# jmschrei/blueberry

Hardware: AMD Instinct MI355X
Metric: Gpair-updates/s per stress iteration, N=50k (higher is better)
Workload: dtype f32

## Files before the change

blueberry_amd/_lib.py:

```python
import ctypes
import os

_HERE = os.path.dirname(os.path.abspath(__file__))
LIB_PATH = os.environ.get("BB_LIB") or os.path.join(_HERE, "libblueberry_hip.so")

BB_OK, BB_ERR_INVALID, BB_ERR_HIP, BB_ERR_STATE, BB_ERR_NOMEM = 0, 1, 2, 3, 4
BB_F32, BB_F64 = 0, 1
BB_KIND_WISH, BB_KIND_COUNTS = 0, 1
BB_PEER_HANDLE_BYTES = 128

c_i32, c_i64, c_dbl = ctypes.c_int32, ctypes.c_int64, ctypes.c_double
p_i32, p_i64, p_dbl = (ctypes.POINTER(c_i32), ctypes.POINTER(c_i64), ctypes.POINTER(c_dbl))
c_int, c_void_p = ctypes.c_int, ctypes.c_void_p


class LayoutInfo(ctypes.Structure):
    _fields_ = [(name, c_i64) for name in (
        "n_bins", "n_pad", "vw", "rows_per_unit", "units_per_tile", "n_blocks", "n_tiles",
        "n_units")]

    def as_dict(self):
        return {name: int(getattr(self, name)) for name, _ in self._fields_}


SIGNATURES = {
    "bb_version": (c_int, []),
    "bb_last_error": (ctypes.c_char_p, []),
    "bb_device_count": (c_int, [ctypes.POINTER(c_int)]),
    "bb_band_count": (c_int, [p_dbl, c_i64, c_i32, c_i32, c_int, p_i64]),
    "bb_band_count_rows": (c_int, [p_dbl, c_i64, c_i32, c_i32, c_i64, c_i64, c_int, p_i64]),
    "bb_layout_dense_info": (c_int, [c_i64, c_int, ctypes.POINTER(LayoutInfo)]),
    "bb_layout_dense_tiles": (c_int, [c_i64, c_int, p_i32, p_i32, c_i64]),
    "bb_layout_rank_units": (c_int, [c_i64, c_int, c_int, p_i64, p_i64]),
    "bb_solver_create": (c_int, [ctypes.POINTER(c_void_p), c_i64, c_int, c_int, c_int, c_int,
                                 p_i32, p_i32, c_i64]),
    "bb_solver_destroy": (c_int, [c_void_p]),
    "bb_solver_set_stream": (c_int, [c_void_p, c_void_p]),
    "bb_solver_layout": (c_int, [c_void_p, ctypes.POINTER(LayoutInfo), p_i64, p_i64]),
    "bb_solver_set_wish_dense": (c_int, [c_void_p, p_dbl, c_i64, c_int, c_dbl]),
    "bb_solver_set_wish_sparse": (c_int, [c_void_p, p_i64, p_i64, p_dbl, c_i64, c_int, c_dbl,
                                          p_dbl, p_dbl]),
    "bb_triples_create": (c_int, [ctypes.POINTER(c_void_p), p_dbl, c_i64, c_i32, c_i32, c_int]),
    "bb_triples_destroy": (c_int, [c_void_p]),
    "bb_triples_tiles": (c_int, [c_void_p, c_i64, c_int, ctypes.POINTER(ctypes.c_uint8), c_i64]),
    "bb_solver_set_wish_triples": (c_int, [c_void_p, c_void_p, c_int, c_dbl, p_dbl, p_dbl]),
    "bb_solver_set_wish_from_coords": (c_int, [c_void_p, p_dbl]),
    "bb_solver_set_coords": (c_int, [c_void_p, p_dbl]),
    "bb_solver_get_coords": (c_int, [c_void_p, p_dbl]),
    "bb_solver_set_momentum": (c_int, [c_void_p, c_dbl]),
    "bb_solver_iterate": (c_int, [c_void_p, c_i64, c_dbl]),
    "bb_solver_grad": (c_int, [c_void_p]),
    "bb_solver_apply": (c_int, [c_void_p, c_dbl]),
    "bb_comm_unique_id": (c_int, [c_void_p]),
    "bb_solver_comm_init": (c_int, [c_void_p, c_void_p]),
    "bb_solver_allreduce": (c_int, [c_void_p]),
    "bb_solver_iterate_dist": (c_int, [c_void_p, c_i64, c_dbl]),
    "bb_solver_peer_export": (c_int, [c_void_p, c_void_p]),
    "bb_solver_peer_connect": (c_int, [c_void_p, c_void_p]),
    "bb_solver_iterate_peer": (c_int, [c_void_p, c_i64, c_dbl]),
    "bb_solver_peer_status": (c_int, [c_void_p, ctypes.POINTER(c_int)]),
    "bb_solver_peer_set_timeout": (c_int, [c_void_p, c_i64]),
    "bb_solver_peer_form": (c_int, [c_void_p, ctypes.POINTER(c_int)]),
    "bb_solver_peer_set_form": (c_int, [c_void_p, c_int]),
    "bb_group_create": (c_int, [ctypes.POINTER(c_void_p), ctypes.POINTER(c_void_p), c_int]),
    "bb_group_iterate": (c_int, [c_void_p, c_i64, c_dbl]),
    "bb_group_destroy": (c_int, [c_void_p]),
    "bb_solver_comm_world": (c_int, [c_void_p, ctypes.POINTER(c_int)]),
    "bb_solver_comm_abort": (c_int, [c_void_p]),
    "bb_comm_cached": (c_int, [c_int, c_int, c_int, ctypes.POINTER(c_int)]),
    "bb_comm_cached_generation": (c_int, [c_int, c_int, c_int, ctypes.POINTER(c_int),
                                          ctypes.POINTER(ctypes.c_uint64)]),
    "bb_solver_comm_attach": (c_int, [c_void_p]),
    "bb_solver_comm_detach": (c_int, [c_void_p]),
    "bb_comm_cache_clear": (c_int, []),
    "bb_solver_sync_timeout": (c_int, [c_void_p, c_i64]),
    "bb_solver_exchange_size": (c_int, [c_void_p, p_i64]),
    "bb_solver_get_exchange_buffer": (c_int, [c_void_p, ctypes.POINTER(c_void_p)]),
    "bb_solver_set_exchange_buffer": (c_int, [c_void_p, c_void_p]),
    "bb_solver_read_exchange": (c_int, [c_void_p, p_dbl, c_i64]),
    "bb_solver_write_exchange": (c_int, [c_void_p, p_dbl, c_i64]),
    "bb_solver_matvec_sq": (c_int, [c_void_p, p_dbl, p_dbl]),
    "bb_solver_spectral_init": (c_int, [c_void_p, c_int, p_dbl]),
    "bb_solver_spectral_init_tol": (c_int, [c_void_p, c_int, c_dbl, p_dbl, ctypes.POINTER(c_int), p_dbl]),
    "bb_solver_stress": (c_int, [c_void_p, p_dbl]),
    "bb_solver_get_stress_history": (c_int, [c_void_p, p_dbl, c_i64, p_i64]),
    "bb_solver_sync": (c_int, [c_void_p]),
    "bb_solver_set_timing": (c_int, [c_void_p, c_int]),
    "bb_solver_get_timing": (c_int, [c_void_p, p_dbl, p_dbl, p_i64]),
    "bb_solver_get_step_timing": (c_int, [c_void_p, p_dbl]),
    "bb_solver_measure_event_gap": (c_int, [c_void_p, c_int, p_dbl]),
    "bb_solver_measure_stream_read": (c_int, [c_void_p, c_int, p_dbl]),
    "bb_solver_iteration_path": (c_int, [c_void_p, ctypes.POINTER(c_int), ctypes.POINTER(c_int)]),
    "bb_solver_traffic": (c_int, [c_void_p, p_i64, p_i64]),
    "bb_cm_create": (c_int, [ctypes.POINTER(c_void_p), c_i64, c_int]),
    "bb_cm_destroy": (c_int, [c_void_p]),
    "bb_cm_dim": (c_int, [c_void_p, p_i64]),
    "bb_cm_device_ptr": (c_int, [c_void_p, ctypes.POINTER(c_void_p), p_i64, ctypes.POINTER(c_int)]),
    "bb_cm_upload": (c_int, [c_void_p, p_dbl, c_i64]),
    "bb_cm_download": (c_int, [c_void_p, p_dbl, c_i64]),
    "bb_cm_scatter": (c_int, [c_void_p, p_dbl, c_i64, c_i32]),
    "bb_cm_scatter_ex": (c_int, [c_void_p, p_dbl, c_i64, c_i32, c_i32, ctypes.POINTER(ctypes.c_uint8),
                                 ctypes.POINTER(c_i32)]),
    "bb_cm_normalize": (c_int, [c_void_p, c_i64, p_dbl, p_dbl]),
    "bb_cm_marginals": (c_int, [c_void_p, p_dbl]),
    "bb_cm_filter": (c_int, [c_void_p, c_dbl, p_i64, ctypes.POINTER(ctypes.c_uint8)]),
    "bb_cm_symv": (c_int, [c_void_p, p_dbl, p_dbl]),
    "bb_cm_eigenvector": (c_int, [c_void_p, p_dbl, p_dbl, c_dbl, c_i64, p_i64, p_dbl]),
    "bb_cm_correlation": (c_int, [c_void_p, p_dbl]),
    "bb_cm_release_scratch": (c_int, [c_int]),
    "bb_cm_shortest_paths": (c_int, [c_void_p, c_void_p, c_int, c_dbl, p_i64]),
    "bb_cm_balance": (c_int, [c_void_p, c_i64, c_i64, c_i64, c_dbl, c_i64, c_dbl, p_dbl,
                              ctypes.POINTER(ctypes.c_uint8), p_i64, p_dbl]),
    "bb_cm_expected": (c_int, [c_void_p, c_i64, p_dbl, p_dbl, p_i64]),
    "bb_triples_balance": (c_int, [c_void_p, c_i64, c_i64, c_i64, c_dbl, c_i64, c_dbl, p_dbl,
                                   ctypes.POINTER(ctypes.c_uint8), p_i64, p_dbl]),
    "bb_triples_expected": (c_int, [c_void_p, c_i64, p_dbl, p_dbl, p_i64]),
    "bb_triples_pairs": (c_int, [c_void_p, c_i64, p_i64]),
    "bb_binomial_sf": (c_int, [p_i64, c_dbl, p_dbl, p_dbl, c_i64, c_int]),
    "bb_cm_significance": (c_int, [c_void_p, c_i64, c_i64, c_i64, p_dbl, c_dbl, c_dbl, p_dbl, c_dbl,
                                   ctypes.POINTER(c_void_p)]),
    "bb_triples_significance": (c_int, [c_void_p, c_i64, c_i64, c_i64, p_dbl, c_dbl, c_dbl, p_dbl,
                                        c_dbl, ctypes.POINTER(c_void_p)]),
    "bb_sig_size": (c_int, [c_void_p, p_i64, p_i64]),
    "bb_sig_read": (c_int, [c_void_p, p_i32, p_i32, p_dbl, p_dbl]),
    "bb_sig_timing": (c_int, [c_void_p, p_dbl, p_dbl]),
    "bb_sig_destroy": (c_int, [c_void_p]),
    "bb_solver_set_wish_from_cm": (c_int, [c_void_p, c_void_p, c_int, c_dbl]),
    "bb_solver_set_wish_from_cm_block": (c_int, [c_void_p, c_void_p, c_i64, c_int, c_dbl]),
    "bb_solver_set_maps": (c_int, [c_void_p, c_int, p_i64, p_dbl]),
    "bb_solver_set_wish_dense_block": (c_int, [c_void_p, p_dbl, c_i64, c_i64, c_i64, c_int, c_dbl]),
    "bb_solver_stress_maps": (c_int, [c_void_p, p_dbl, c_int]),
    "bb_solver_set_block_steps": (c_int, [c_void_p, p_dbl, c_i64]),
    "bb_solver_set_bin_steps": (c_int, [c_void_p, p_dbl, c_i64]),
    "bb_solver_degrees": (c_int, [c_void_p, p_i64, c_i64]),
    "bb_solver_set_weight_power": (c_int, [c_void_p, c_int]),
    "bb_solver_weight_sums": (c_int, [c_void_p, p_dbl, c_i64]),
    "bb_solver_score": (c_int, [c_void_p, p_dbl, p_dbl, p_dbl]),
    "bb_solver_get_score_timing": (c_int, [c_void_p, p_dbl, p_dbl, p_dbl]),
    "bb_contactmap_scatter": (c_int, [p_dbl, c_i64, c_i32, p_dbl, c_i64, c_int]),
    "bb_contactmap_normalize": (c_int, [p_dbl, c_i64, p_dbl, p_dbl, c_int]),
    "bb_benjamini_hochberg": (c_int, [p_dbl, c_i64, c_i64, p_dbl, c_int]),
    "bb_downsample": (c_int, [ctypes.POINTER(ctypes.c_float), c_i64,
                              ctypes.POINTER(ctypes.c_float), c_i64, c_int]),
}

_lib = None


def load():
    global _lib
    if _lib is not None:
        return _lib
    if not os.path.exists(LIB_PATH):
        raise ImportError(
            "blueberry_amd: %s is missing -- build it with `python -c 'import __graft_entry__ as "
            "g; g.build()'` (or ./build.sh) at the repository root. There is no CPU fallback."
            % LIB_PATH)
    lib = ctypes.CDLL(LIB_PATH)
    for name, (restype, argtypes) in SIGNATURES.items():
        fn = getattr(lib, name)
        fn.restype = restype
        fn.argtypes = argtypes
    _lib = lib
    return lib


def hip_runtimes_loaded():
    paths = set()
    try:
        with open("/proc/self/maps") as fh:
            for line in fh:
                if "libamdhip64" in line:
                    paths.add(line.split()[-1])
    except OSError:
        pass
    return sorted(paths)
# ... 21 lines not shown
```

blueberry_amd/csrc/bb_solver.hip:

```cpp
#include <math.h>
#include <stddef.h>
#include <stdlib.h>
#include <string.h>
#include <time.h>
#include <unistd.h>

#include <algorithm>
#include <cmath>
#include <type_traits>
#include <vector>

#include <condition_variable>
#include <map>
#include <mutex>
#include <thread>
#include <tuple>

#include "bb_comm.h"
#include "bb_common.h"
#include "bb_group_barrier.h"
#include "bb_score.h"
#include "bb_solver_kernels.h"
#include "bb_triples.h"

struct bb_solver {
    int dtype = BB_F32, device = 0, rank = 0, world = 1;
    bool wide = true;
    bb_layout_info L{};
    std::vector<int32_t> tile_I, tile_J;
    int64_t u_begin = 0, u_end = 0, n_local = 0;
    int64_t t_first = 0, n_local_tiles = 0;
    std::vector<int2> udesc;

    hipStream_t stream = nullptr;
    bool own_stream = false;
    bool stream_stuck = false;

    void *d_units = nullptr, *d_X = nullptr, *d_V = nullptr, *d_part = nullptr;
    void *d_exch = nullptr;
    bb::DevBuf own_exch;
    double momentum = 0.0;
    int2 *d_udesc = nullptr;
    int chunk_q = 0, chunk_r = 0;
    bool nontemporal = true;
    bb::DevBuf d_arena;
    int2 *d_wave_slots = nullptr;
    int lds_wave_floats = 0;
    double *d_stresspart = nullptr;
    double *d_stress_slot = nullptr;
    std::vector<int32_t> slot_strip;
    std::vector<int32_t> wave_last_strip;
    int n_maps = 1;
    bb::DevBuf d_bin_scale;
    bb::DevBuf d_map_ptr, d_map_idx;
    bb::DevBuf d_map_scalar;
    std::vector<int64_t> map_begin;
    int64_t *d_red_lists = nullptr;
    int red_stride = 0, red_slices = 0;
    double *d_stress_hist = nullptr, *d_stress_scalar = nullptr;
    double *d_f64_tmp = nullptr;
    bb::DevBuf d_mv_in;
    int64_t rowpart_elems = 0, colpart_elems = 0;
    int n_waves = 0, n_slots = 0;
    int wpb = 4;
    int dense_u0 = -1;
    int defer_cap_units = 0;
    int64_t defer_lds_bytes = 0;
    unsigned defer_attr_done = 0;
    int64_t hist_cap = 0, hist_n = 0;
    bool have_wish = false, have_coords = false, grad_pending = false;
    void *sum_target = nullptr;

    bb::Rccl::Comm comm = nullptr;
    bool comm_cached = false;
    bool comm_suspect = false;

    bb::DevBuf peer_arena;
    int64_t peer_slot_elems = 0, peer_arena_bytes = 0;
    std::vector<void *> peer_mapped;
    std::vector<void *> peer_opened;
    bb::DevBuf d_peer_table;
    bb::DevBuf d_peer_table_x;
    bool peer_fused = true;
    bb::DevBuf d_peer_state;
    int peer_clock_khz = 100000;
    int peer_ranks_on_gpu = 1;
    bb::DevBuf d_peer_mask;
    bb::DevBuf d_peer_counter;
    unsigned long long peer_seq = 0;
    long long peer_limit_ticks = 0;
    bool peer_connected = false;

    bool row_owner = false;
    bool row_owner_built = false;
    bool bin_steps = false;
    int weight_power = 0;
    void *d_full = nullptr, *d_X2 = nullptr;
    int64_t full_ld = 0;
    double *d_ro_part = nullptr;
    int ro_blocks = 0, ro_wpr = 1;
    int64_t ro_launches = 0;

    bool timing = false;
    int timing_stride = 1;
    int64_t timing_iter = 0;
    std::vector<bb::Event> ev;
    size_t ev_used = 0;
    double score_ms[3] = {0.0, 0.0, 0.0};
};

namespace {

void comm_release(bb_solver *s, bool destroy);

constexpr int64_t kHistCap = 1 << 20;
constexpr size_t kMaxTimedLaunches = 4096;

int check_kind_alpha(const char *who, int kind, double alpha) {
    BB_REQUIRE(kind == BB_KIND_WISH || kind == BB_KIND_COUNTS, std::string(who) + ": bad kind");
    BB_REQUIRE(kind == BB_KIND_WISH || alpha > 0.0, std::string(who) + ": alpha must be > 0");
    return BB_OK;
}

hipError_t upload_padded(const bb_solver *s, double *dst, const double *rows, hipStream_t stream) {
    const hipError_t e = hipMemsetAsync(dst, 0, (size_t)s->L.n_pad * 3 * sizeof(double), stream);
    if (e != hipSuccess) return e;
    return hipMemcpyAsync(dst, rows, (size_t)s->L.n_bins * 3 * sizeof(double), hipMemcpyHostToDevice, stream);
}

int enable_peer_access(const char *who, int device) {
    const hipError_t e = hipDeviceEnablePeerAccess(device, 0);
    if (e != hipSuccess && e != hipErrorPeerAccessAlreadyEnabled) return bb::hip_status(who, e);
    (void)hipGetLastError();
    return BB_OK;
}

template <typename TearDown>
int failed_create(int rc, TearDown &&tear_down) {
    const std::string keep = bb_last_error();
    tear_down();
    bb::set_error(keep);
    return rc;
}

int64_t peer_flags_offset(const bb_solver *s) {
    return 2 * (int64_t)s->world * s->peer_slot_elems * bb::elem_size(s->dtype);
}
int64_t peer_xpoison_offset(const bb_solver *s) {
    return peer_flags_offset(s) + bb::round_up((int64_t)s->world * 64, 256);
}
int64_t peer_arena_size(const bb_solver *s) {
    return peer_xpoison_offset(s) + bb::round_up((int64_t)s->world * 64, 256);
}

int waves_per_cu(int64_t n_local) {
    const char *e = getenv("BB_WAVES_PER_CU");
    int v = e ? atoi(e) : (n_local >= 65000 ? 8 : 4);
    if (v < 1) v = 1;
    if (v > 32) v = 32;
    return v;
}

int64_t row_owner_max() {
    const char *e = getenv("BB_ROW_OWNER_MAX");
    return e ? atoll(e) : bb::kRowOwnerMaxBins;
}

int build_indices(bb_solver *s) {
    const int64_t upt = s->L.units_per_tile, vw = s->L.vw;
    const int64_t ch = 3 * vw;
    s->n_local = s->u_end - s->u_begin;
    s->t_first = s->n_local > 0 ? s->u_begin / upt : 0;
    const int64_t t_last = s->n_local > 0 ? (s->u_end - 1) / upt : -1;
    s->n_local_tiles = s->n_local > 0 ? t_last - s->t_first + 1 : 0;

    s->udesc.resize((size_t)std::max<int64_t>(s->n_local, 1));
    for (int64_t ul = 0; ul < s->n_local; ++ul) {
        const int64_t u = s->u_begin + ul, t = u / upt, sub = u % upt;
        s->udesc[ul] = make_int2((int)(s->tile_I[t] * vw + sub * s->L.rows_per_unit),
                                 (int)(s->tile_J[t] * vw));
    }

    int cus = 256;
    hipDeviceGetAttribute(&cus, hipDeviceAttributeMultiprocessorCount, s->device);
    int64_t want = (int64_t)cus * waves_per_cu(s->n_local);
    int64_t nw = std::max<int64_t>(1, std::min<int64_t>(want, s->n_local));
    {
        const char *e = getenv("BB_PAIR");
        const bool pair = !(e && atoi(e) == 0);
        s->wpb = (pair && (s->dtype == BB_F32 || s->wide) && waves_per_cu(s->n_local) >= 8 && nw >= 8)
                     ? 8 : 4;
    }
    nw = bb::round_up(nw, s->wpb);
    s->n_waves = (int)nw;

    if (s->n_local >= ((int64_t)1 << 31))
        return bb::fail(BB_ERR_INVALID, "bb_solver_create: more than 2^31 units on one rank");
    s->nontemporal = s->n_local * bb::kUnitBytes > ((int64_t)240 << 20);
    s->chunk_q = (int)(s->n_local / nw);
    s->chunk_r = (int)(s->n_local % nw);
    std::vector<int2> wave_range(nw);
    int64_t chunk_max = 0;
    for (int64_t w = 0; w < nw; ++w) {
        const int64_t a = w * s->chunk_q + std::min<int64_t>(w, s->chunk_r);
        wave_range[w] = make_int2((int)a, (int)(a + s->chunk_q + (w < s->chunk_r ? 1 : 0)));
        chunk_max = std::max<int64_t>(chunk_max, wave_range[w].y - wave_range[w].x);
    }
    {
        const int64_t wgs_per_cu = std::max<int64_t>(1, (nw / s->wpb + cus - 1) / cus);
        const int64_t budget = 156 * 1024 / wgs_per_cu;
        const int64_t cap = std::min<int64_t>(chunk_max, (budget / s->wpb - 16 - 8) / 48);
        if ((s->dtype == BB_F32 || s->wide) && cap > 0) s->defer_cap_units = (int)cap;
        const int64_t col_words = 3 * vw * bb::elem_size(s->dtype) / 4;
        s->lds_wave_floats = (int)std::max<int64_t>((int64_t)s->defer_cap_units * 12 + 4, col_words);
        s->defer_lds_bytes = (int64_t)s->wpb * s->lds_wave_floats * 4 + 32;
    }
    std::vector<int32_t> &slot_strip = s->slot_strip;
    slot_strip.clear();
    s->wave_last_strip.assign((size_t)nw, -1);
    std::vector<int2> wave_slots(nw);
    for (int64_t w = 0; w < nw; ++w) {
        wave_slots[w] = make_int2((int)slot_strip.size(), -1);
        if (wave_range[w].x >= wave_range[w].y) continue;
        int cur = -1;
        std::vector<int> strips;
        for (int64_t ul = wave_range[w].x; ul < wave_range[w].y; ++ul) {
            const int J = s->udesc[ul].y / (int)vw;
            if (J != cur) { strips.push_back(J); cur = J; }
        }
        for (size_t q = 0; q + 1 < strips.size(); ++q) slot_strip.push_back(strips[q]);
        const int Jlast = strips.back();
        s->wave_last_strip[(size_t)w] = Jlast;
        const bool same_wg = w % s->wpb != 0;
        if (same_wg && wave_slots[w - 1].y >= 0 &&
            slot_strip[(size_t)wave_slots[w - 1].y] == Jlast) {
            wave_slots[w].y = wave_slots[w - 1].y;
        } else {
            wave_slots[w].y = (int)slot_strip.size();
            slot_strip.push_back(Jlast);
        }
    }
    s->n_slots = (int)slot_strip.size();
    s->rowpart_elems = s->n_local_tiles * ch;
    s->colpart_elems = (int64_t)s->n_slots * ch;

    const int64_t nb = s->L.n_blocks;
    std::vector<int64_t> blk_ptr(nb + 1, 0);
    for (int64_t lt = 0; lt < s->n_local_tiles; ++lt) blk_ptr[s->tile_I[s->t_first + lt] + 1]++;
    for (int sl = 0; sl < s->n_slots; ++sl) blk_ptr[slot_strip[sl] + 1]++;
    for (int64_t b = 0; b < nb; ++b) blk_ptr[b + 1] += blk_ptr[b];
    std::vector<int64_t> blk_chunk((size_t)std::max<int64_t>(blk_ptr[nb], 1));
    std::vector<int64_t> fill(blk_ptr.begin(), blk_ptr.end() - 1);
    for (int64_t lt = 0; lt < s->n_local_tiles; ++lt)
        blk_chunk[fill[s->tile_I[s->t_first + lt]]++] = lt * ch;
    for (int sl = 0; sl < s->n_slots; ++sl)
        blk_chunk[fill[slot_strip[sl]]++] = s->rowpart_elems + (int64_t)sl * ch;

    int64_t longest = 0;
    for (int64_t b = 0; b < nb; ++b) longest = std::max(longest, blk_ptr[b + 1] - blk_ptr[b]);
    const int64_t zero_off = s->rowpart_elems + s->colpart_elems;
    const int64_t part_total = zero_off + ch;
    std::vector<int64_t> red_lists;
    {
        s->red_slices = longest <= 64 ? 4 : 8;
        if (const char *f = getenv("BB_REDUCE_SLICES")) s->red_slices = atoi(f) == 4 ? 4 : 8;
        const int64_t quantum = 16 * s->red_slices;
        s->red_stride = (int)bb::round_up(std::max<int64_t>(longest, 1), quantum);
        red_lists.assign((size_t)(nb * s->red_stride), zero_off);
        for (int64_t b = 0; b < nb; ++b)
            for (int64_t k = blk_ptr[b]; k < blk_ptr[b + 1]; ++k)
                red_lists[(size_t)(b * s->red_stride + (k - blk_ptr[b]))] = blk_chunk[k];
    }

    const int64_t es = bb::elem_size(s->dtype);
    s->hist_cap = kHistCap;
    if (s->row_owner) {
        s->full_ld = bb::round_up(s->L.n_bins, s->dtype == BB_F32 ? RowTrip<float>::COLS
                                                                  : RowTrip<double>::COLS);
        s->ro_wpr = s->L.n_bins <= 1024 ? 4 : (s->L.n_bins <= 2048 ? 2 : 1);
        const int rows_per_wg = 4 / s->ro_wpr;
        s->ro_blocks = (int)((s->L.n_bins + rows_per_wg - 1) / rows_per_wg);
// ... 1 lines not shown
    {
        std::vector<std::pair<void **, size_t>> want;
        auto add = [&](auto **ptr, int64_t count) {
            want.push_back({(void **)ptr, (size_t)std::max<int64_t>(count, 1) * sizeof(**ptr)});
        };
        add((char **)&s->d_units, std::max<int64_t>(s->n_local, 1) * bb::kUnitBytes);
        add((char **)&s->d_X, s->L.n_pad * 3 * es);
        add((char **)&s->d_V, s->L.n_pad * 3 * es);
        add((char **)&s->d_part, part_total * es);
        add(&s->d_udesc, (int64_t)s->udesc.size());
        add(&s->d_wave_slots, nw);
        add(&s->d_stresspart, nw);
        add(&s->d_stress_slot, std::max<int64_t>(s->n_slots, 1));
        add(&s->d_red_lists, (int64_t)red_lists.size());
        add(&s->d_stress_hist, kHistCap);
        add(&s->d_stress_scalar, 1);
        add(&s->d_f64_tmp, s->L.n_pad * 3);
        if (s->row_owner) {
            add((char **)&s->d_full, s->L.n_bins * s->full_ld * es);
            add((char **)&s->d_X2, s->L.n_pad * 3 * es);
            add(&s->d_ro_part, 2 * (int64_t)s->ro_blocks);
        }
        size_t total = 0;
        for (auto &w : want) total += (w.second + 255) & ~(size_t)255;
        BB_TRY(bb::alloc_status(s->d_arena, total));
        size_t off = 0;
        for (auto &w : want) {
            *w.first = s->d_arena.as<char>() + off;
            off += (w.second + 255) & ~(size_t)255;
        }
    }
    BB_TRY(bb::alloc_status(s->own_exch, (size_t)((3 * s->L.n_pad + 2) * es)));
    s->d_exch = s->own_exch.p;

    hipStream_t st = s->stream;
    BB_HIP_CHECK(hipMemcpyAsync(s->d_udesc, s->udesc.data(), s->udesc.size() * sizeof(int2),
                                hipMemcpyHostToDevice, st));
    BB_HIP_CHECK(hipMemcpyAsync(s->d_wave_slots, wave_slots.data(), nw * sizeof(int2),
                                hipMemcpyHostToDevice, st));
    BB_HIP_CHECK(hipMemcpyAsync(s->d_red_lists, red_lists.data(),
                                red_lists.size() * sizeof(int64_t), hipMemcpyHostToDevice, st));
    BB_HIP_CHECK(hipMemsetAsync(s->d_part, 0, (size_t)part_total * es, st));
    BB_HIP_CHECK(hipMemsetAsync(s->d_X, 0, (size_t)(s->L.n_pad * 3 * es), st));
    BB_HIP_CHECK(hipMemsetAsync(s->d_V, 0, (size_t)(s->L.n_pad * 3 * es), st));
    if (s->row_owner)
        BB_HIP_CHECK(hipMemsetAsync(s->d_X2, 0, (size_t)(s->L.n_pad * 3 * es), st));
    BB_HIP_CHECK(hipMemsetAsync(s->d_exch, 0, (size_t)((3 * s->L.n_pad + 2) * es), st));
    BB_HIP_CHECK(hipMemsetAsync(s->d_stresspart, 0, (size_t)nw * sizeof(double), st));
    BB_HIP_CHECK(hipMemsetAsync(s->d_stress_slot, 0,
                                (size_t)std::max<int64_t>(s->n_slots, 1) * sizeof(double), st));
    BB_HIP_CHECK(hipStreamSynchronize(st));
    return BB_OK;
}

template <typename TT>
struct TypeTag {
    using T = TT;
};
template <typename TT, bool WW>
struct LayoutTag {
    using T = TT;
    static constexpr bool W = WW;
};

template <typename F>
decltype(auto) by_layout(const bb_solver *s, F &&f) {
    if (s->dtype == BB_F32) return f(LayoutTag<float, true>{});
    if (s->wide) return f(LayoutTag<double, true>{});
    return f(LayoutTag<double, false>{});
}

template <typename F>
decltype(auto) by_dtype(const bb_solver *s, F &&f) {
    if (s->dtype == BB_F32) return f(TypeTag<float>{});
    return f(TypeTag<double>{});
}

template <int V, int... Rest, typename F>
decltype(auto) with_int(int v, F &&f) {
    if constexpr (sizeof...(Rest) == 0) return f(std::integral_constant<int, V>{});
    else return v == V ? f(std::integral_constant<int, V>{}) : with_int<Rest...>(v, f);
}

template <bool NT, int OP, int WPB, typename T, bool W>
int launch_sweep(LayoutTag<T, W>, bb_solver *s, const void *x_in) {
    const auto kern = stress_grad_kernel<T, W, NT, OP, WPB>;
    constexpr unsigned bit = 1u << ((WPB == 8 ? 4 : 0) + (NT ? 2 : 0) + (OP == kOpMatvec2 ? 1 : 0) +
                                    (OP == kOpStressW1 ? 8 : 0) + (OP == kOpStressW2 ? 16 : 0));
    if (s->defer_lds_bytes > 0 && !(s->defer_attr_done & bit)) {
        BB_HIP_CHECK(hipFuncSetAttribute((const void *)kern, hipFuncAttributeMaxDynamicSharedMemorySize,
                                         (int)s->defer_lds_bytes));
        s->defer_attr_done |= bit;
    }
    T *rowpart = (T *)s->d_part +
                 (s->u_begin - s->t_first * s->L.units_per_tile) * (3 * s->L.rows_per_unit);
    T *colpart = (T *)s->d_part + s->rowpart_elems;
    BB_HIP_CHECK(bb::launch(kern, dim3(s->n_waves / s->wpb), dim3(64 * s->wpb), (size_t)s->defer_lds_bytes,
                            s->stream, (const T *)s->d_units, (const T *)x_in, s->d_udesc, s->chunk_q,
                            s->chunk_r, s->d_wave_slots, rowpart, colpart, s->d_stresspart,
                            s->defer_cap_units, s->lds_wave_floats, s->dense_u0, s->d_stress_slot));
    return BB_OK;
}

template <int OP, typename L>
int launch_sweep_op(L lay, bb_solver *s, const void *x_in) {
    constexpr int kPairWpb = sizeof(typename L::T) == 4 || L::W ? 8 : 4;
    return with_int<1, 0>(s->nontemporal ? 1 : 0, [&](auto nt) {
        return with_int<kPairWpb, 4>(s->wpb, [&](auto wpb) {
            return launch_sweep<decltype(nt)::value != 0, OP, decltype(wpb)::value>(lay, s, x_in);
        });
    });
}

constexpr double kScaleGradient = 2.0, kScalePlainSum = 1.0;

template <typename T>
void fill_reduce_params(bb_solver *s, ReduceParams<T> &p, int mode, double lr, double *stress_out,
                        double scale);

template <typename T, bool W>
int launch_exchange_t(LayoutTag<T, W>, bb_solver *s, double lr, double *stress_out, double scale) {
    ReduceParams<T> p;
    fill_reduce_params<T>(s, p, kReducePeer, lr, stress_out, scale);
    const int64_t es = sizeof(T);
    const unsigned segs = 3 * Lay<T, W>::VW / kRedWG;
    const dim3 grid((unsigned)s->L.n_blocks, segs);
    const PeerTableX<T> *xt = s->d_peer_table_x.as<const PeerTableX<T>>() + (s->peer_seq & 1);
    const char *base = s->peer_arena.as<const char>();
    const T *arena = (const T *)(base + (int64_t)(s->peer_seq & 1) * s->world * s->peer_slot_elems * es);
    const unsigned long long *my_poison = (const unsigned long long *)(base + peer_xpoison_offset(s));
    return with_int<4, 8>(s->red_slices, [&](auto slices) -> int {
        constexpr int S = decltype(slices)::value;
        BB_HIP_CHECK(bb::launch(reduce_exchange_kernel<T, W, S>, grid, dim3(128 * S), 0, s->stream, p,
                                (const int64_t *)s->d_red_lists, s->red_stride, xt, arena, my_poison,
                                s->peer_slot_elems, s->d_peer_state.as<PeerState>(),
                                s->peer_limit_ticks));
        return BB_OK;
    });
}

template <typename T>
void fill_reduce_params(bb_solver *s, ReduceParams<T> &p, int mode, double lr, double *stress_out,
                        double scale) {
    p.part = (const T *)s->d_part;
    p.stresspart = s->d_stresspart;
    p.X = s->sum_target ? (T *)s->sum_target : (T *)s->d_X;
    p.V = (T *)s->d_V;
    p.mu = s->sum_target ? T(0) : (T)s->momentum;
    p.scale = (T)scale;
    p.exch = (T *)s->d_exch;
    p.stress_out = stress_out;
    p.n_pad = s->L.n_pad;
    p.n_waves = s->n_waves;
    p.lr = s->sum_target ? T(-1) : (T)lr;
    p.peer = nullptr;
    p.peer_counter = s->d_peer_counter.as<unsigned>();
    p.peer_state = s->d_peer_state.as<PeerState>();
    p.seq = 0;
    p.n_peers = 0;
    if (mode == kReducePeer) {
        p.peer = s->d_peer_table.as<const PeerTable<T>>() + (s->peer_seq & 1);
        p.seq = s->peer_seq;
        p.n_peers = s->world;
    }
    p.mode = mode;
    p.stress_slot = s->d_stress_slot;
    p.n_slots = s->n_slots;
    p.bin_scale = scale == kScalePlainSum ? nullptr : s->d_bin_scale.as<const T>();
    p.map_ptr = s->d_map_ptr.as<int>();
    p.map_idx = s->d_map_idx.as<int>();
    p.n_maps = s->n_maps;
    p.peer_mask = s->d_peer_mask.as<unsigned>();
    p.rank = s->rank;
}

template <typename T, bool W>
int launch_reduce_t(LayoutTag<T, W>, bb_solver *s, int mode, double lr, double *stress_out, double scale) {
    ReduceParams<T> p;
    fill_reduce_params<T>(s, p, mode, lr, stress_out, scale);
    const unsigned segs = 3 * Lay<T, W>::VW / kRedWG;
    const dim3 grid = mode == kReduceStressOnly ? dim3((unsigned)s->n_maps, 1)
// ... 95 lines not shown
            std::max<int64_t>(0, std::min<int64_t>(i_start + rows, n) - i_start);
        const int64_t cols_valid =
            std::max<int64_t>(0, std::min<int64_t>((int64_t)j0 + VW, n) - j0);
        hipError_t e = hipSuccess;
        if (rows_valid < rows || cols_valid < VW)
            e = hipMemsetAsync(stage, 0, (size_t)rows * VW * sizeof(double), s->stream);
        if (e == hipSuccess && rows_valid > 0 && cols_valid > 0)
            e = hipMemcpy2DAsync(stage, VW * sizeof(double), host + (i_start - off) * ld + (j0 - off),
                                 (size_t)ld * sizeof(double), (size_t)cols_valid * sizeof(double),
                                 (size_t)rows_valid, hipMemcpyHostToDevice, s->stream);
        if (e == hipSuccess) {
            e = bb::launch(convert_units_kernel<T, W>, dim3((unsigned)(ue - ul)), dim3(256), 0,
                           s->stream, stage, (T *)s->d_units, s->d_udesc, ul, i_start, n, kind,
                           -1.0 / alpha);
        }
        if (e != hipSuccess)
            rc = bb::hip_status("set_wish_dense", e);
        ul = ue;
    }
    hipError_t e = hipStreamSynchronize(s->stream);
    if (rc == BB_OK && e != hipSuccess)
        rc = bb::hip_status("set_wish_dense", e);
    return rc;
}

int upload_bin_scale(bb_solver *s, const double *padded) {
    const int64_t n = s->L.n_pad, es = bb::elem_size(s->dtype);
    std::vector<char> host((size_t)(n * es));
    for (int64_t i = 0; i < n; ++i) {
        if (s->dtype == BB_F32) ((float *)host.data())[i] = (float)padded[i];
        else ((double *)host.data())[i] = padded[i];
    }
    BB_HIP_CHECK(hipStreamSynchronize(s->stream));
    if (!s->d_bin_scale) BB_TRY(bb::alloc_status(s->d_bin_scale, (size_t)(n * es)));
    BB_HIP_CHECK(hipMemcpy(s->d_bin_scale.p, host.data(), host.size(), hipMemcpyHostToDevice));
    return BB_OK;
}

int refresh_full(bb_solver *s) {
    if (!s->row_owner) return BB_OK;
    const int64_t es = bb::elem_size(s->dtype);
    BB_HIP_CHECK(hipMemsetAsync(s->d_full, 0, (size_t)(s->L.n_bins * s->full_ld * es), s->stream));
    if (s->n_local > 0)
        BB_TRY(by_layout(s, [&](auto lay) -> int {
            using T = typename decltype(lay)::T;
            BB_HIP_CHECK(bb::launch(units_to_full_kernel<T, decltype(lay)::W>, dim3((unsigned)s->n_local),
                                    dim3(256), 0, s->stream, (const T *)s->d_units, s->d_udesc,
                                    (T *)s->d_full, s->full_ld, s->L.n_bins));
            return BB_OK;
        }));
    BB_HIP_CHECK(hipStreamSynchronize(s->stream));
    return BB_OK;
}

int launch_row_owner(bb_solver *s, double lr, bool fold_prev, bool update) {
    const int par = (int)(s->ro_launches & 1);
    const double *prev = s->d_ro_part + (int64_t)(par ^ 1) * s->ro_blocks;
    double *out = s->d_ro_part + (int64_t)par * s->ro_blocks;
    double *hist_prev = fold_prev ? s->d_stress_hist + (s->hist_n - 1) : nullptr;
    const unsigned grid = update ? (unsigned)s->ro_blocks + 1u : 1u;
    BB_TRY(by_dtype(s, [&](auto t) {
        using T = typename decltype(t)::T;
        return with_int<4, 2, 1>(s->ro_wpr, [&](auto wpr) {
            return with_int<1, 2, 0>(s->weight_power, [&](auto q) -> int {
                BB_HIP_CHECK(bb::launch(row_owner_kernel<T, decltype(wpr)::value, decltype(q)::value>,
                                        dim3(grid), dim3(256), 0, s->stream, (const T *)s->d_full,
                                        s->full_ld, (int)s->L.n_bins, (const T *)s->d_X, (T *)s->d_X2,
                                        (T *)s->d_V, (T)lr, (T)s->momentum, prev, s->ro_blocks, hist_prev,
                                        out, s->d_bin_scale.as<const T>()));
                return BB_OK;
            });
        });
    }));
    if (update) {
        std::swap(s->d_X, s->d_X2);
        s->ro_launches++;
    }
    return BB_OK;
}

int inputs_done(bb_solver *s) {
    BB_HIP_CHECK(hipStreamSynchronize(s->stream));
    BB_TRY(refresh_full(s));
    s->have_wish = true;
    return BB_OK;
}

int pack_from_cm(bb_solver *s, const double *m, int64_t d, int64_t off, int kind, double alpha) {
    BB_TRY(bb::enter_device(s->device));
    if (s->n_local > 0)
        BB_TRY(by_layout(s, [&](auto lay) -> int {
            using T = typename decltype(lay)::T;
            BB_HIP_CHECK(bb::launch(pack_units_from_matrix_kernel<T, decltype(lay)::W>,
                                    dim3((unsigned)s->n_local), dim3(256), 0, s->stream, m, d,
                                    (T *)s->d_units, s->d_udesc, off + d, kind, -1.0 / alpha, off));
            return BB_OK;
        }));
    return inputs_done(s);
}

int set_wish_dense(bb_solver *s, const double *host, int64_t ld, int kind, double alpha, int64_t off,
                   int64_t n_sub) {
    BB_TRY(bb::enter_device(s->device));
    BB_TRY(by_layout(s, [&](auto lay) { return set_wish_dense_t(lay, s, host, ld, kind, alpha, off, n_sub); }));
    return inputs_done(s);
}

template <typename Stage>
int scatter_entries(bb_solver *s, const char *who, int64_t n, int64_t chunk, int kind, double alpha,
                    const double *KRnorm, const double *KRexpected, Stage &&stage) {
    const auto hip = [&](hipError_t e) { return bb::hip_status(who, e); };
    const int64_t nb = s->L.n_blocks;
    std::vector<int32_t> tilemap((size_t)(nb * nb), -1);
    for (size_t t = 0; t < s->tile_I.size(); ++t)
        tilemap[(size_t)s->tile_I[t] * nb + s->tile_J[t]] = (int32_t)t;
    bb::DevBuf bmap, bbad, bkr, bke;
    if (bmap.alloc(tilemap.size() * 4) != hipSuccess || bbad.alloc(sizeof(int)) != hipSuccess ||
        (KRnorm && (bkr.alloc((size_t)s->L.n_bins * 8) != hipSuccess ||
                    bke.alloc((size_t)s->L.n_bins * 8) != hipSuccess)))
        return bb::fail(BB_ERR_NOMEM, std::string(who) + ": out of device memory");
    hipStream_t st = s->stream;
    BB_TRY(hip(hipMemcpyAsync(bmap.p, tilemap.data(), tilemap.size() * 4, hipMemcpyHostToDevice, st)));
    if (KRnorm) {
        BB_TRY(hip(hipMemcpyAsync(bkr.p, KRnorm, (size_t)s->L.n_bins * 8, hipMemcpyHostToDevice, st)));
        BB_TRY(hip(hipMemcpyAsync(bke.p, KRexpected, (size_t)s->L.n_bins * 8, hipMemcpyHostToDevice, st)));
    }
    BB_TRY(hip(hipMemsetAsync(bbad.p, 0, sizeof(int), st)));
    BB_TRY(hip(hipMemsetAsync(s->d_units, 0, (size_t)std::max<int64_t>(s->n_local, 1) * bb::kUnitBytes, st)));
    for (int64_t k0 = 0; k0 < n; k0 += chunk) {
        const int64_t m = std::min(chunk, n - k0);
        EntrySrc src;
        BB_TRY(hip(stage(k0, m, &src)));
        for (int ph = 0; ph < 3; ++ph)
            BB_TRY(hip(by_layout(s, [&](auto lay) {
                using T = typename decltype(lay)::T;
                return bb::launch(scatter_entries_kernel<T, decltype(lay)::W>, dim3((unsigned)((m + 255) / 256)),
                                  dim3(256), 0, st, src, m, (const int32_t *)bmap.p, nb, s->L.n_bins,
                                  s->u_begin, s->u_end, (T *)s->d_units, kind, -1.0 / alpha,
                                  (const double *)bkr.p, (const double *)bke.p, (int *)bbad.p, ph);
            })));
    }
    BB_TRY(hip(hipStreamSynchronize(st)));
    int bad = 0;
    BB_TRY(hip(hipMemcpy(&bad, bbad.p, sizeof(int), hipMemcpyDeviceToHost)));
    if (bad == 1)
        return bb::fail(BB_ERR_INVALID, std::string(who) + ": an index is outside [0, n_bins)");
    if (bad == 2)
        return bb::fail(BB_ERR_INVALID, std::string(who) + ": an entry falls in a tile that is not in "
                                                           "the solver's tile list");
    return inputs_done(s);
}

}

namespace {

struct PeerHandle {
    hipIpcMemHandle_t ipc;
    uint64_t magic;
    int64_t arena_bytes, slot_elems;
    int64_t pid;
    uint64_t raw;
    int32_t rank, world, dtype, device;
    uint64_t pci;
};
static_assert(sizeof(PeerHandle) <= BB_PEER_HANDLE_BYTES, "handle blob too small");
static_assert(offsetof(PeerTable<float>, flag) == kMaxPeers * sizeof(void *) &&
                  offsetof(PeerTable<double>, flag) == kMaxPeers * sizeof(void *),
              "peer_receive_kernel takes the flag pointers as the second half of a PeerTable");
constexpr uint64_t kPeerMagic = 0x6262706565723031ull;

int contributor_mask(const bb_solver *s, std::vector<unsigned> *mask) {
    mask->assign((size_t)s->L.n_blocks, 0u);
    const int64_t upt = s->L.units_per_tile;
    for (int q = 0; q < s->world; ++q) {
        int64_t ub = 0, ue = 0;
        BB_TRY(bb_layout_rank_units(s->L.n_units, q, s->world, &ub, &ue));
        if (ue <= ub) continue;
        for (int64_t t = ub / upt; t <= (ue - 1) / upt; ++t) {
            (*mask)[(size_t)s->tile_I[(size_t)t]] |= 1u << q;
            (*mask)[(size_t)s->tile_J[(size_t)t]] |= 1u << q;
        }
    }
    return BB_OK;
}

template <typename T>
int build_peer_tables(TypeTag<T>, bb_solver *s) {
    PeerTable<T> tab[2];
    memset(tab, 0, sizeof(tab));
    const int64_t foff = peer_flags_offset(s);
    for (int par = 0; par < 2; ++par)
        for (int q = 0; q < s->world; ++q) {
            char *base = (char *)s->peer_mapped[q];
            tab[par].dst[q] = (T *)base + ((int64_t)par * s->world + s->rank) * s->peer_slot_elems;
            tab[par].flag[q] = (unsigned long long *)(base + foff) + 8 * s->rank;
        }
    BB_TRY(bb::alloc_status(s->d_peer_table, sizeof(tab)));
    BB_HIP_CHECK(hipMemcpy(s->d_peer_table.p, tab, sizeof(tab), hipMemcpyHostToDevice));
    PeerTableX<T> tx[2];
    memset(tx, 0, sizeof(tx));
    for (int par = 0; par < 2; ++par)
        for (int q = 0; q < s->world; ++q) {
            char *base = (char *)s->peer_mapped[q];
            tx[par].dst[q] = tab[par].dst[q];
            tx[par].poison[q] = (unsigned long long *)(base + peer_xpoison_offset(s)) + 8 * s->rank;
        }
    BB_TRY(bb::alloc_status(s->d_peer_table_x, sizeof(tx)));
    BB_HIP_CHECK(hipMemcpy(s->d_peer_table_x.p, tx, sizeof(tx), hipMemcpyHostToDevice));
// ... 82 lines not shown
        }
    }
    for (void *m : s->peer_opened) hipIpcCloseMemHandle(m);
    const int device = s->device;
    hipStream_t pooled = s->own_stream && !s->stream_stuck ? s->stream : nullptr;
    delete s;
    if (pooled) bb::release_stream(device, pooled);
    (void)hipGetLastError();
    return BB_OK;
}

int bb_solver_set_stream(bb_solver *s, void *hip_stream) {
    BB_REQUIRE(s != nullptr, "bb_solver_set_stream: solver is NULL");
    BB_TRY(bb::enter_device(s->device));
    BB_HIP_CHECK(hipStreamSynchronize(s->stream));
    if (s->own_stream && s->stream) bb::release_stream(s->device, s->stream);
    s->stream = (hipStream_t)hip_stream;
    s->own_stream = false;
    return BB_OK;
}

int bb_solver_layout(const bb_solver *s, bb_layout_info *info, int64_t *u_begin, int64_t *u_end) {
    BB_REQUIRE(s != nullptr, "bb_solver_layout: solver is NULL");
    if (info) *info = s->L;
    if (u_begin) *u_begin = s->u_begin;
    if (u_end) *u_end = s->u_end;
    return BB_OK;
}

int bb_solver_set_wish_dense(bb_solver *s, const double *host, int64_t ld, int kind,
                             double alpha) {
    BB_REQUIRE(s != nullptr && host != nullptr, "bb_solver_set_wish_dense: NULL argument");
    BB_REQUIRE(ld >= s->L.n_bins, "bb_solver_set_wish_dense: ld < n_bins");
    BB_TRY(check_kind_alpha("bb_solver_set_wish_dense", kind, alpha));
    return set_wish_dense(s, host, ld, kind, alpha, 0, s->L.n_bins);
}

int bb_solver_set_maps(bb_solver *s, int n_maps, const int64_t *bin_begin, const double *lr_scale) {
    BB_REQUIRE(s != nullptr && bin_begin != nullptr && lr_scale != nullptr,
               "bb_solver_set_maps: NULL argument");
    BB_REQUIRE(n_maps >= 1 && n_maps <= s->L.n_blocks, "bb_solver_set_maps: bad n_maps");
    if (s->world != 1)
        return bb::fail(BB_ERR_STATE, "bb_solver_set_maps: one rank only (on several GPUs give every "
                                      "rank maps of its own)");
    const int64_t vw = s->L.vw, nb = s->L.n_blocks;
    BB_REQUIRE(bin_begin[0] == 0 && bin_begin[n_maps] == s->L.n_bins,
               "bb_solver_set_maps: bin_begin must run from 0 to n_bins");
    for (int m = 0; m < n_maps; ++m)
        BB_REQUIRE(bin_begin[m] % vw == 0 && bin_begin[m + 1] > bin_begin[m],
                   "bb_solver_set_maps: every map starts at a multiple of the tile edge and is not empty");
    BB_TRY(bb::enter_device(s->device));
    std::vector<int> map_of_block((size_t)nb, 0);
    for (int m = 0, b = 0; b < nb; ++b) {
        while (m + 1 < n_maps && (int64_t)b * vw >= bin_begin[m + 1]) ++m;
        map_of_block[(size_t)b] = m;
    }
    for (size_t t = 0; t < s->tile_I.size(); ++t)
        BB_REQUIRE(map_of_block[(size_t)s->tile_I[t]] == map_of_block[(size_t)s->tile_J[t]],
                   "bb_solver_set_maps: a tile of the solver's list joins two maps");
    std::vector<double> scale((size_t)s->L.n_pad);
    for (int64_t i = 0; i < s->L.n_pad; ++i) scale[(size_t)i] = lr_scale[map_of_block[(size_t)(i / vw)]];
    std::vector<std::vector<int>> lists((size_t)n_maps);
    for (int w = 0; w < s->n_waves; ++w)
        if (s->wave_last_strip[(size_t)w] >= 0)
            lists[(size_t)map_of_block[(size_t)s->wave_last_strip[(size_t)w]]].push_back(w);
    for (int q = 0; q < s->n_slots; ++q)
        lists[(size_t)map_of_block[(size_t)s->slot_strip[(size_t)q]]].push_back(s->n_waves + q);
    std::vector<int> ptr(1, 0), idx;
    for (auto &l : lists) {
        idx.insert(idx.end(), l.begin(), l.end());
        ptr.push_back((int)idx.size());
    }
    if (idx.empty()) idx.push_back(0);
    s->d_bin_scale.reset(); s->d_map_ptr.reset(); s->d_map_idx.reset(); s->d_map_scalar.reset();
    s->bin_steps = false;
    s->n_maps = 1;
    s->map_begin.clear();
    BB_TRY(upload_bin_scale(s, scale.data()));
    BB_TRY(bb::alloc_status(s->d_map_ptr, ptr.size() * sizeof(int)));
    BB_TRY(bb::alloc_status(s->d_map_idx, idx.size() * sizeof(int)));
    BB_TRY(bb::alloc_status(s->d_map_scalar, (size_t)n_maps * sizeof(double)));
    BB_HIP_CHECK(hipMemcpy(s->d_map_ptr.p, ptr.data(), ptr.size() * sizeof(int), hipMemcpyHostToDevice));
    BB_HIP_CHECK(hipMemcpy(s->d_map_idx.p, idx.data(), idx.size() * sizeof(int), hipMemcpyHostToDevice));
    BB_HIP_CHECK(hipMemsetAsync(s->d_units, 0, (size_t)std::max<int64_t>(s->n_local, 1) * bb::kUnitBytes,
                                s->stream));
    BB_HIP_CHECK(hipStreamSynchronize(s->stream));
    s->n_maps = n_maps;
    s->map_begin.assign(bin_begin, bin_begin + n_maps + 1);
    s->row_owner = false;
    s->hist_n = 0;
    return BB_OK;
}

int bb_solver_set_bin_steps(bb_solver *s, const double *scale, int64_t n_bins) {
    BB_REQUIRE(s != nullptr, "bb_solver_set_bin_steps: solver is NULL");
    if (s->n_maps > 1 && scale == nullptr)
        return bb::fail(BB_ERR_STATE, "bb_solver_set_bin_steps: a solver of several maps always has "
                                      "factors (bb_solver_set_maps sets each map's; pass new ones)");
    if (s->grad_pending)
        return bb::fail(BB_ERR_STATE, "bb_solver_set_bin_steps: a bb_solver_grad is pending");
    BB_TRY(bb::enter_device(s->device));
    if (scale == nullptr) {
        BB_HIP_CHECK(hipStreamSynchronize(s->stream));
        s->d_bin_scale.reset();
        s->bin_steps = false;
        return BB_OK;
    }
    BB_REQUIRE(n_bins == s->L.n_bins, "bb_solver_set_bin_steps: one factor per bin");
    std::vector<double> padded((size_t)s->L.n_pad, 1.0);
    for (int64_t i = 0; i < n_bins; ++i) {
        BB_REQUIRE(std::isfinite(scale[i]) && scale[i] > 0.0,
                   "bb_solver_set_bin_steps: factors must be finite and positive");
        padded[(size_t)i] = scale[i];
    }
    BB_TRY(upload_bin_scale(s, padded.data()));
    s->bin_steps = true;
    return BB_OK;
}

int bb_solver_set_block_steps(bb_solver *s, const double *scale, int64_t n_blocks) {
    BB_REQUIRE(s != nullptr, "bb_solver_set_block_steps: solver is NULL");
    if (scale == nullptr) return bb_solver_set_bin_steps(s, nullptr, 0);
    BB_REQUIRE(n_blocks == s->L.n_blocks, "bb_solver_set_block_steps: one factor per block of the "
                                          "layout (bb_solver_layout: n_blocks)");
    std::vector<double> per_bin((size_t)s->L.n_bins);
    for (int64_t i = 0; i < s->L.n_bins; ++i) per_bin[(size_t)i] = scale[i / s->L.vw];
    return bb_solver_set_bin_steps(s, per_bin.data(), s->L.n_bins);
}

int bb_solver_degrees(bb_solver *s, int64_t *degree, int64_t n_bins) {
    BB_REQUIRE(s != nullptr && degree != nullptr, "bb_solver_degrees: NULL argument");
    BB_REQUIRE(n_bins == s->L.n_bins, "bb_solver_degrees: one count per bin");
    if (!s->have_wish) return bb::fail(BB_ERR_STATE, "bb_solver_degrees: no wish distances set");
    BB_TRY(bb::enter_device(s->device));
    int *d_deg = (int *)s->d_f64_tmp;
    BB_HIP_CHECK(hipMemsetAsync(d_deg, 0, (size_t)s->L.n_pad * sizeof(int), s->stream));
    if (s->n_local > 0)
        BB_TRY(by_layout(s, [&](auto lay) -> int {
            using T = typename decltype(lay)::T;
            BB_HIP_CHECK(bb::launch(unit_degrees_kernel<T, decltype(lay)::W>,
                                    dim3((unsigned)((s->n_local + kDegUnits - 1) / kDegUnits)), dim3(256),
                                    0, s->stream, (const T *)s->d_units, s->d_udesc, s->n_local,
                                    s->L.n_bins, d_deg));
            return BB_OK;
        }));
    std::vector<int> host((size_t)n_bins);
    BB_HIP_CHECK(hipStreamSynchronize(s->stream));
    BB_HIP_CHECK(hipMemcpy(host.data(), d_deg, (size_t)n_bins * sizeof(int), hipMemcpyDeviceToHost));
    for (int64_t i = 0; i < n_bins; ++i) degree[i] = host[(size_t)i];
    return BB_OK;
}

int bb_solver_set_weight_power(bb_solver *s, int q) {
    BB_REQUIRE(s != nullptr, "bb_solver_set_weight_power: solver is NULL");
    BB_REQUIRE(q >= 0 && q <= 2, "bb_solver_set_weight_power: q must be 0, 1 or 2");
    if (s->grad_pending)
        return bb::fail(BB_ERR_STATE, "bb_solver_set_weight_power: a bb_solver_grad is pending");
    s->weight_power = q;
    return BB_OK;
}

int bb_solver_weight_sums(bb_solver *s, double *sums, int64_t n_bins) {
    BB_REQUIRE(s != nullptr && sums != nullptr, "bb_solver_weight_sums: NULL argument");
    BB_REQUIRE(n_bins == s->L.n_bins, "bb_solver_weight_sums: one sum per bin");
    if (!s->have_wish) return bb::fail(BB_ERR_STATE, "bb_solver_weight_sums: no wish distances set");
    BB_TRY(bb::enter_device(s->device));
// ... 134 lines not shown

int bb_triples_create(bb_triples **out, const double *triples, int64_t n, int32_t resolution,
                      int32_t row_major, int device) {
    BB_REQUIRE(out != nullptr, "bb_triples_create: out is NULL");
    *out = nullptr;
    BB_REQUIRE(n >= 0 && (n == 0 || triples != nullptr), "bb_triples_create: NULL triples");
    BB_REQUIRE(resolution > 0, "bb_triples_create: resolution must be positive");
    BB_TRY(bb::use_device(device));
    bb_triples *t = new (std::nothrow) bb_triples();
    if (!t) return bb::fail(BB_ERR_NOMEM, "bb_triples_create: out of host memory");
    t->device = device;
    t->n = n;
    t->resolution = (double)resolution;
    if (row_major) { t->st = 3; t->sc = 1; } else { t->st = 1; t->sc = n; }
    int rc = bb::alloc_status(t->d, (size_t)(3 * n) * sizeof(double));
    if (rc == BB_OK && n > 0)
        rc = bb::hip_status("bb_triples_create",
                            hipMemcpy(t->d.p, triples, (size_t)n * 24, hipMemcpyHostToDevice));
    if (rc != BB_OK) {
        delete t;
        return rc;
    }
    *out = t;
    return BB_OK;
}

int bb_triples_destroy(bb_triples *t) {
    if (!t) return BB_OK;
    hipSetDevice(t->device);
    delete t;
    (void)hipGetLastError();
    return BB_OK;
}

int bb_triples_tiles(const bb_triples *t, int64_t n_bins, int dtype, uint8_t *present,
                     int64_t n_blocks) {
    BB_REQUIRE(t != nullptr && present != nullptr, "bb_triples_tiles: NULL argument");
    bb_layout_info L;
    BB_TRY(bb_layout_dense_info(n_bins, dtype, &L));
    BB_REQUIRE(n_blocks == L.n_blocks, "bb_triples_tiles: present must hold n_blocks^2 bytes of "
                                       "the layout of (n_bins, dtype)");
    BB_TRY(bb::enter_device(t->device));
    bb::DevBuf bp, bb_;
    if (bp.alloc((size_t)(n_blocks * n_blocks)) != hipSuccess || bb_.alloc(sizeof(int)) != hipSuccess)
        return bb::fail(BB_ERR_NOMEM, "bb_triples_tiles: out of device memory");
    BB_HIP_CHECK(hipMemset(bp.p, 0, (size_t)(n_blocks * n_blocks)));
    BB_HIP_CHECK(hipMemset(bb_.p, 0, sizeof(int)));
    constexpr int64_t kChunk = (int64_t)1 << 30;
    for (int64_t k0 = 0; k0 < t->n; k0 += kChunk) {
        const int64_t m = std::min(kChunk, t->n - k0);
        const EntrySrc src = {nullptr, nullptr, nullptr, t->from(k0), t->st, t->sc, t->resolution};
        BB_HIP_CHECK(bb::launch(entries_tiles_kernel, dim3((unsigned)((m + 255) / 256)), dim3(256), 0,
                                (hipStream_t) nullptr, src, m, L.vw, n_blocks, n_bins,
                                (unsigned char *)bp.p, (int *)bb_.p));
    }
    int bad = 0;
    BB_HIP_CHECK(hipMemcpy(&bad, bb_.p, sizeof(int), hipMemcpyDeviceToHost));
    BB_HIP_CHECK(hipMemcpy(present, bp.p, (size_t)(n_blocks * n_blocks), hipMemcpyDeviceToHost));
    if (bad) return bb::fail(BB_ERR_INVALID, "bb_triples_tiles: an index is outside [0, n_bins)");
    return BB_OK;
}

int bb_solver_set_wish_triples(bb_solver *s, const bb_triples *t, int kind, double alpha,
                               const double *KRnorm, const double *KRexpected) {
    BB_REQUIRE(s != nullptr && t != nullptr, "bb_solver_set_wish_triples: NULL argument");
    BB_TRY(check_kind_alpha("bb_solver_set_wish_triples", kind, alpha));
    BB_REQUIRE((KRnorm == nullptr) == (KRexpected == nullptr),
               "bb_solver_set_wish_triples: KRnorm and KRexpected go together");
    BB_REQUIRE(t->device == s->device,
               "bb_solver_set_wish_triples: the triples live on another device than the solver");
    BB_TRY(bb::enter_device(s->device));
    constexpr int64_t kChunk = (int64_t)1 << 30;
    return scatter_entries(s, "bb_solver_set_wish_triples", t->n, kChunk, kind, alpha, KRnorm, KRexpected,
                           [&](int64_t k0, int64_t, EntrySrc *src) {
        *src = {nullptr, nullptr, nullptr, t->from(k0), t->st, t->sc, t->resolution};
        return hipSuccess;
    });
}

int bb_solver_set_wish_from_coords(bb_solver *s, const double *xstar) {
    BB_REQUIRE(s != nullptr && xstar != nullptr, "bb_solver_set_wish_from_coords: NULL argument");
    BB_TRY(bb::enter_device(s->device));
    BB_HIP_CHECK(upload_padded(s, s->d_f64_tmp, xstar, s->stream));
    if (s->n_local > 0)
        BB_TRY(by_layout(s, [&](auto lay) -> int {
            using T = typename decltype(lay)::T;
            BB_HIP_CHECK(bb::launch(gen_units_kernel<T, decltype(lay)::W>, dim3((unsigned)s->n_local),
                                    dim3(256), 0, s->stream, s->d_f64_tmp, (T *)s->d_units, s->d_udesc,
                                    s->L.n_bins));
            return BB_OK;
        }));
    return inputs_done(s);
}

int bb_solver_set_coords(bb_solver *s, const double *xyz) {
    BB_REQUIRE(s != nullptr && xyz != nullptr, "bb_solver_set_coords: NULL argument");
    BB_TRY(bb::enter_device(s->device));
    const int64_t n3 = s->L.n_pad * 3;
    BB_HIP_CHECK(upload_padded(s, s->d_f64_tmp, xyz, s->stream));
    BB_HIP_CHECK(narrow(s, s->d_f64_tmp, s->d_X, n3));
    BB_HIP_CHECK(hipMemsetAsync(s->d_V, 0, (size_t)n3 * bb::elem_size(s->dtype), s->stream));
    BB_HIP_CHECK(hipStreamSynchronize(s->stream));
    s->have_coords = true;
    s->hist_n = 0;
    s->grad_pending = false;
    return BB_OK;
}

int bb_solver_get_coords(bb_solver *s, double *xyz) {
    BB_REQUIRE(s != nullptr && xyz != nullptr, "bb_solver_get_coords: NULL argument");
    if (!s->have_coords) return bb::fail(BB_ERR_STATE, "bb_solver_get_coords: no coordinates set");
    BB_TRY(bb::enter_device(s->device));
    const int64_t n3 = s->L.n_pad * 3;
    BB_HIP_CHECK(widen(s, s->d_X, s->d_f64_tmp, n3));
    BB_HIP_CHECK(hipStreamSynchronize(s->stream));
    BB_HIP_CHECK(hipMemcpy(xyz, s->d_f64_tmp, (size_t)s->L.n_bins * 3 * sizeof(double),
                           hipMemcpyDeviceToHost));
    return BB_OK;
}

int bb_solver_set_momentum(bb_solver *s, double mu) {
    BB_REQUIRE(s != nullptr, "bb_solver_set_momentum: solver is NULL");
    BB_REQUIRE(mu >= 0.0 && mu < 1.0, "bb_solver_set_momentum: need 0 <= mu < 1");
    s->momentum = mu;
    return BB_OK;
}

int bb_solver_iterate(bb_solver *s, int64_t iters, double lr) {
    BB_TRY(check_iterate(s, iters, "bb_solver_iterate"));
    if (s->world != 1)
        return bb::fail(BB_ERR_STATE,
                        "bb_solver_iterate: world > 1 needs bb_solver_grad / all-reduce / "
                        "bb_solver_apply");
    BB_TRY(bb::enter_device(s->device));
    if (s->row_owner) {
        for (int64_t k = 0; k < iters; ++k) {
            BB_TRY(timed_step(s, [&] { return launch_row_owner(s, lr, k > 0, true); },
                              [] { return (int)BB_OK; }));
            s->hist_n++;
        }
        if (iters > 0) BB_TRY(launch_row_owner(s, lr, true, false));
        return BB_OK;
    }
    for (int64_t k = 0; k < iters; ++k) {
        BB_TRY(timed_step(s, [&] { return launch_grad(s); }, [&] {
            return launch_reduce(s, kReduceApply, lr, s->d_stress_hist + s->hist_n * s->n_maps);
        }));
        s->hist_n++;
    }
    return BB_OK;
}

int bb_solver_grad(bb_solver *s) {
    BB_TRY(check_ready(s, "bb_solver_grad"));
    if (s->n_maps > 1)
        return bb::fail(BB_ERR_STATE, "bb_solver_grad: a solver of several maps (bb_solver_set_maps) "
                                      "iterates with bb_solver_iterate only");
    BB_TRY(bb::enter_device(s->device));
    BB_TRY(timed_step(s, [&] { return launch_grad(s); },
                      [&] { return launch_reduce(s, kReduceExchange, 0.0, nullptr); }));
    s->grad_pending = true;
    return BB_OK;
}

int bb_solver_apply(bb_solver *s, double lr) {
    BB_TRY(check_ready(s, "bb_solver_apply"));
// ... 296 lines not shown
    h.device = s->device;
    {
        int dom = 0, bus = 0, dev = 0;
        if (hipDeviceGetAttribute(&dom, hipDeviceAttributePciDomainID, s->device) != hipSuccess ||
            hipDeviceGetAttribute(&bus, hipDeviceAttributePciBusId, s->device) != hipSuccess ||
            hipDeviceGetAttribute(&dev, hipDeviceAttributePciDeviceId, s->device) != hipSuccess) {
            (void)hipGetLastError();
            dom = bus = dev = 0;
        }
        h.pci = ((uint64_t)(uint32_t)dom << 32) | ((uint64_t)(bus & 0xffff) << 16) | (uint64_t)(dev & 0xffff);
    }
    memset(handle_out, 0, BB_PEER_HANDLE_BYTES);
    memcpy(handle_out, &h, sizeof(h));
    return BB_OK;
}

int bb_solver_peer_connect(bb_solver *s, const void *handles) {
    BB_REQUIRE(s != nullptr && handles != nullptr, "bb_solver_peer_connect: NULL argument");
    if (!s->peer_arena) return bb::fail(BB_ERR_STATE, "bb_solver_peer_connect: export first");
    if (s->peer_connected) return bb::fail(BB_ERR_STATE, "bb_solver_peer_connect: already connected");
    BB_TRY(bb::enter_device(s->device));
    s->peer_mapped.assign((size_t)s->world, nullptr);
    std::map<uint64_t, int> ranks_on_gpu;
    int most_on_one_gpu = 1;
    for (int r = 0; r < s->world; ++r) {
        PeerHandle h;
        memcpy(&h, (const char *)handles + (size_t)r * BB_PEER_HANDLE_BYTES, sizeof(h));
        most_on_one_gpu = std::max(most_on_one_gpu, ++ranks_on_gpu[h.pci]);
        if (h.magic != kPeerMagic || h.rank != r || h.world != s->world || h.dtype != s->dtype ||
            h.arena_bytes != s->peer_arena_bytes || h.slot_elems != s->peer_slot_elems)
            return bb::fail(BB_ERR_INVALID, "bb_solver_peer_connect: handle " + std::to_string(r) +
                                                " does not match this solver (rank order, world, "
                                                "dtype and n_bins must agree)");
        if (r == s->rank) {
            s->peer_mapped[r] = s->peer_arena.p;
        } else if (h.pid == (int64_t)getpid()) {
            if (h.device != s->device)
                BB_TRY(enable_peer_access("bb_solver_peer_connect: peer access", h.device));
            s->peer_mapped[r] = (void *)(uintptr_t)h.raw;
        } else {
            void *ptr = nullptr;
            hipError_t e = hipIpcOpenMemHandle(&ptr, h.ipc, hipIpcMemLazyEnablePeerAccess);
            if (e != hipSuccess)
                return bb::fail(BB_ERR_HIP, "bb_solver_peer_connect: hipIpcOpenMemHandle(rank " +
                                                std::to_string(r) + "): " + hipGetErrorString(e));
            s->peer_mapped[r] = ptr;
            s->peer_opened.push_back(ptr);
        }
    }
    BB_TRY(by_dtype(s, [&](auto t) { return build_peer_tables(t, s); }));
    {
        const char *env = getenv("BB_PEER_MASK");
        s->d_peer_mask.reset();
        if (!(env && atoi(env) == 0) && s->world <= 32) {
            std::vector<unsigned> mask;
            BB_TRY(contributor_mask(s, &mask));
            BB_TRY(bb::alloc_status(s->d_peer_mask, mask.size() * sizeof(unsigned)));
            BB_HIP_CHECK(hipMemcpy(s->d_peer_mask.p, mask.data(), mask.size() * sizeof(unsigned),
                                   hipMemcpyHostToDevice));
        }
    }
    BB_TRY(bb::alloc_status(s->d_peer_state, sizeof(PeerState)));
    const int64_t n_counters = 32 * (s->L.n_blocks + 1);
    BB_TRY(bb::alloc_status(s->d_peer_counter, (size_t)n_counters * sizeof(unsigned)));
    BB_HIP_CHECK(hipMemset(s->d_peer_state.p, 0, sizeof(PeerState)));
    BB_HIP_CHECK(hipMemset(s->d_peer_counter.p, 0, (size_t)n_counters * sizeof(unsigned)));
    int khz = 0;
    if (hipDeviceGetAttribute(&khz, hipDeviceAttributeWallClockRate, s->device) != hipSuccess) {
        (void)hipGetLastError();
        khz = 0;
    }
    s->peer_clock_khz = khz > 0 ? khz : 100000;
    long long ms = 10000;
    if (const char *env = getenv("BB_PEER_TIMEOUT_MS")) {
        const long long v = atoll(env);
        if (v > 0) ms = v;
    }
    s->peer_limit_ticks = ms * s->peer_clock_khz;
    s->peer_seq = 0;
    {
        const char *env = getenv("BB_PEER_FUSED");
        s->peer_fused = env ? atoi(env) != 0 : most_on_one_gpu == 1;
        s->peer_ranks_on_gpu = most_on_one_gpu;
    }
    s->peer_connected = true;
    BB_HIP_CHECK(hipDeviceSynchronize());
    return BB_OK;
}

int bb_solver_peer_set_timeout(bb_solver *s, int64_t milliseconds) {
    BB_REQUIRE(s != nullptr, "bb_solver_peer_set_timeout: solver is NULL");
    BB_REQUIRE(milliseconds > 0 && milliseconds <= 3600000,
               "bb_solver_peer_set_timeout: need 0 < ms <= 3600000");
    if (!s->peer_connected)
        return bb::fail(BB_ERR_STATE, "bb_solver_peer_set_timeout: not connected");
    s->peer_limit_ticks = (long long)milliseconds * s->peer_clock_khz;
    return BB_OK;
}

int bb_solver_peer_set_form(bb_solver *s, int one_launch) {
    BB_REQUIRE(s != nullptr, "bb_solver_peer_set_form: solver is NULL");
    if (!s->peer_connected)
        return bb::fail(BB_ERR_STATE, "bb_solver_peer_set_form: not connected");
    if (s->peer_seq != 0)
        return bb::fail(BB_ERR_STATE, "bb_solver_peer_set_form: exchanges have already run");
    s->peer_fused = one_launch != 0;
    return BB_OK;
}

int bb_solver_peer_form(bb_solver *s, int *one_launch) {
    BB_REQUIRE(s != nullptr && one_launch != nullptr, "bb_solver_peer_form: NULL argument");
    if (!s->peer_connected) return bb::fail(BB_ERR_STATE, "bb_solver_peer_form: not connected");
    *one_launch = s->peer_fused ? 1 : 0;
    return BB_OK;
}

int bb_solver_peer_status(bb_solver *s, int *status) {
    BB_REQUIRE(s != nullptr, "bb_solver_peer_status: solver is NULL");
    if (!s->peer_connected) return bb::fail(BB_ERR_STATE, "bb_solver_peer_status: not connected");
    BB_TRY(bb::enter_device(s->device));
    PeerState st;
    memset(&st, 0, sizeof(st));
    BB_HIP_CHECK(hipStreamSynchronize(s->stream));
    BB_HIP_CHECK(hipMemcpy(&st, s->d_peer_state.p, sizeof(st), hipMemcpyDeviceToHost));
    if (status) *status = st.status;
    if (st.status != 0) {
        const bool one = s->peer_fused;
        return bb::fail(BB_ERR_STATE,
                        std::string("peer exchange: a rank did not deliver its partial within the "
                                    "time limit (BB_PEER_TIMEOUT_MS), or reported its own failure; ") +
                            (one ? "the last exchange this rank completed whole was "
                                 : "this rank's coordinates were left at its last completed step (") +
                            std::to_string(st.verdict) + " of " + std::to_string(s->peer_seq) +
                            (one ? " (the one after it may be applied in part: the coordinates of "
                                   "this solver are not a result)"
                                 : " exchanges)") +
                            " and every peer has been told to stop");
    }
    return BB_OK;
}

int bb_solver_iterate_peer(bb_solver *s, int64_t iters, double lr) {
    BB_TRY(check_iterate(s, iters, "bb_solver_iterate_peer"));
    if (!s->peer_connected)
        return bb::fail(BB_ERR_STATE, "bb_solver_iterate_peer: bb_solver_peer_connect first");
    if (s->grad_pending)
        return bb::fail(BB_ERR_STATE, "bb_solver_iterate_peer: a bb_solver_grad is pending");
    if (s->n_maps > 1)
        return bb::fail(BB_ERR_STATE, "bb_solver_iterate_peer: a solver of several maps "
                                      "(bb_solver_set_maps) iterates with bb_solver_iterate only");
    BB_TRY(bb::enter_device(s->device));
    for (int64_t k = 0; k < iters; ++k) {
        double *hist = s->d_stress_hist + s->hist_n;
        BB_TRY(timed_step(s, [&] { return launch_grad(s); }, [&] {
            s->peer_seq++;
            return s->peer_fused ? launch_exchange(s, lr, hist) : launch_reduce(s, kReducePeer, 0.0, nullptr);
        }));
        if (!s->peer_fused) BB_TRY(launch_peer_receive(s, s->d_X, lr, s->momentum, hist));
        s->hist_n++;
    }
    return BB_OK;
}

int bb_solver_exchange_size(const bb_solver *s, int64_t *n_elems) {
    BB_REQUIRE(s != nullptr && n_elems != nullptr, "bb_solver_exchange_size: NULL argument");
    *n_elems = 3 * s->L.n_pad + 2;
// ... 143 lines not shown
    BB_HIP_CHECK(hipStreamSynchronize(s->stream));
    if (enabled && s->ev.empty()) {
        s->ev.resize(3 * kMaxTimedLaunches);
        for (bb::Event &e : s->ev) BB_HIP_CHECK(e.create());
    }
    s->timing = enabled != 0;
    s->timing_stride = enabled > 1 ? enabled : 1;
    s->timing_iter = 0;
    s->ev_used = 0;
    return BB_OK;
}

int bb_solver_get_timing(bb_solver *s, double *grad_ms_avg, double *reduce_ms_avg,
                         int64_t *launches) {
    BB_REQUIRE(s != nullptr, "bb_solver_get_timing: solver is NULL");
    BB_TRY(bb::enter_device(s->device));
    BB_HIP_CHECK(hipStreamSynchronize(s->stream));
    double g = 0.0, r = 0.0;
    const size_t n = s->ev_used / 3;
    for (size_t k = 0; k < n; ++k) {
        float a = 0.f, b = 0.f;
        BB_HIP_CHECK(hipEventElapsedTime(&a, s->ev[3 * k], s->ev[3 * k + 1]));
        BB_HIP_CHECK(hipEventElapsedTime(&b, s->ev[3 * k + 1], s->ev[3 * k + 2]));
        g += a;
        r += b;
    }
    if (grad_ms_avg) *grad_ms_avg = n ? g / n : 0.0;
    if (reduce_ms_avg) *reduce_ms_avg = n ? r / n : 0.0;
    if (launches) *launches = (int64_t)n;
    return BB_OK;
}

int bb_solver_get_step_timing(bb_solver *s, double *step_ms_avg) {
    BB_REQUIRE(s != nullptr && step_ms_avg != nullptr, "bb_solver_get_step_timing: NULL argument");
    BB_TRY(bb::enter_device(s->device));
    BB_HIP_CHECK(hipStreamSynchronize(s->stream));
    const size_t n = s->ev_used / 3;
    double t = 0.0;
    for (size_t k = 0; k + 1 < n; ++k) {
        float a = 0.f;
        BB_HIP_CHECK(hipEventElapsedTime(&a, s->ev[3 * k], s->ev[3 * k + 3]));
        t += a;
    }
    *step_ms_avg = n > 1 ? t / (double)(n - 1) / s->timing_stride : 0.0;
    return BB_OK;
}

int bb_solver_measure_event_gap(bb_solver *s, int pairs, double *ms_avg) {
    BB_REQUIRE(s != nullptr && ms_avg != nullptr, "bb_solver_measure_event_gap: NULL argument");
    BB_REQUIRE(pairs >= 1 && pairs <= 256, "bb_solver_measure_event_gap: bad pairs");
    BB_TRY(check_ready(s, "bb_solver_measure_event_gap"));
    BB_TRY(bb::enter_device(s->device));
    std::vector<bb::Event> ev((size_t)2 * pairs);
    hipError_t e = hipSuccess;
    for (bb::Event &x : ev)
        if (e == hipSuccess) e = x.create();
    for (int k = 0; k < pairs && e == hipSuccess; ++k) {
        if (!s->row_owner && launch_grad(s) != BB_OK) e = hipErrorUnknown;
        if (e == hipSuccess) e = hipEventRecord(ev[(size_t)2 * k], s->stream);
        if (e == hipSuccess) e = hipEventRecord(ev[(size_t)2 * k + 1], s->stream);
    }
    if (e == hipSuccess) e = hipStreamSynchronize(s->stream);
    double t = 0.0;
    for (int k = 0; k < pairs && e == hipSuccess; ++k) {
        float a = 0.f;
        e = hipEventElapsedTime(&a, ev[(size_t)2 * k], ev[(size_t)2 * k + 1]);
        t += a;
    }
    if (e != hipSuccess)
        return bb::hip_status("bb_solver_measure_event_gap", e);
    *ms_avg = t / pairs;
    return BB_OK;
}

int bb_solver_measure_stream_read(bb_solver *s, int launches, double *ms_avg) {
    BB_REQUIRE(s != nullptr && ms_avg != nullptr, "bb_solver_measure_stream_read: NULL argument");
    BB_REQUIRE(launches >= 1 && launches <= 1000, "bb_solver_measure_stream_read: bad launches");
    if (!s->have_wish)
        return bb::fail(BB_ERR_STATE, "bb_solver_measure_stream_read: no wish distances set");
    BB_TRY(bb::enter_device(s->device));
    bb::Event e0, e1;
    BB_HIP_CHECK(e0.create());
    BB_HIP_CHECK(e1.create());
    auto launch = [&]() {
        return bb::launch(s->nontemporal ? stream_read_kernel<true> : stream_read_kernel<false>,
                          dim3(s->n_waves / 4), dim3(256), 0, s->stream,
                          (const float4 *)s->d_units, s->chunk_q, s->chunk_r,
                          (float *)s->d_f64_tmp);
    };
    BB_HIP_CHECK(launch());
    BB_HIP_CHECK(hipEventRecord(e0, s->stream));
    for (int k = 0; k < launches; ++k) BB_HIP_CHECK(launch());
    BB_HIP_CHECK(hipEventRecord(e1, s->stream));
    BB_HIP_CHECK(hipEventSynchronize(e1));
    float ms = 0.f;
    BB_HIP_CHECK(hipEventElapsedTime(&ms, e0, e1));
    *ms_avg = ms / launches;
    return BB_OK;
}

int bb_solver_iteration_path(const bb_solver *s, int *row_owner, int *waves_per_row) {
    BB_REQUIRE(s != nullptr, "bb_solver_iteration_path: solver is NULL");
    if (row_owner) *row_owner = s->row_owner ? 1 : 0;
    if (waves_per_row) *waves_per_row = s->row_owner ? s->ro_wpr : 0;
    return BB_OK;
}

int bb_solver_traffic(const bb_solver *s, int64_t *unit_bytes, int64_t *pairs_dense) {
    BB_REQUIRE(s != nullptr, "bb_solver_traffic: solver is NULL");
    if (unit_bytes) *unit_bytes = s->n_local * bb::kUnitBytes;
    if (pairs_dense) *pairs_dense = s->L.n_bins * (s->L.n_bins - 1) / 2;
    return BB_OK;
}

}

namespace {

void jacobi3(double *a, double *z) {
    for (int q = 0; q < 9; ++q) z[q] = (q % 4 == 0) ? 1.0 : 0.0;
    for (int sweep = 0; sweep < 50; ++sweep) {
        const double off = a[1] * a[1] + a[2] * a[2] + a[5] * a[5];
        if (off < 1e-300) break;
        for (int p = 0; p < 3; ++p)
            for (int q = p + 1; q < 3; ++q) {
                const double apq = a[p * 3 + q];
                if (apq == 0.0) continue;
                const double theta = (a[q * 3 + q] - a[p * 3 + p]) / (2.0 * apq);
                const double t = (theta >= 0 ? 1.0 : -1.0) / (fabs(theta) + sqrt(theta * theta + 1.0));
                const double c = 1.0 / sqrt(t * t + 1.0), sn = t * c;
                for (int k = 0; k < 3; ++k) {
                    const double akp = a[k * 3 + p], akq = a[k * 3 + q];
                    a[k * 3 + p] = c * akp - sn * akq;
                    a[k * 3 + q] = sn * akp + c * akq;
                }
                for (int k = 0; k < 3; ++k) {
                    const double apk = a[p * 3 + k], aqk = a[q * 3 + k];
                    a[p * 3 + k] = c * apk - sn * aqk;
                    a[q * 3 + k] = sn * apk + c * aqk;
                }
                for (int k = 0; k < 3; ++k) {
                    const double zkp = z[k * 3 + p], zkq = z[k * 3 + q];
                    z[k * 3 + p] = c * zkp - sn * zkq;
                    z[k * 3 + q] = sn * zkp + c * zkq;
                }
            }
    }
}

template <typename T>
int spectral_init_t(TypeTag<T>, bb_solver *s, int n_iter, const double *v0, double tol, int *iters_done,
                    double *residual_out) {
    const int64_t n = s->L.n_bins, n_pad = s->L.n_pad, n3 = n_pad * 3;
    if (!s->d_mv_in) BB_TRY(bb::alloc_status(s->d_mv_in, (size_t)n3 * sizeof(T)));
    bb::DevBuf bV, bZ, bS, bP, bF;
    if (bV.alloc((size_t)n3 * 8) != hipSuccess || bZ.alloc((size_t)n3 * 8) != hipSuccess ||
        bS.alloc(24 * 8) != hipSuccess || bP.alloc((size_t)2 * kSpMaxGroups * 12 * 8) != hipSuccess ||
        bF.alloc(sizeof(int)) != hipSuccess)
        return bb::fail(BB_ERR_NOMEM, "bb_solver_spectral_init: out of device memory");
    double *dV = (double *)bV.p, *dZ = (double *)bZ.p, *dS = (double *)bS.p;
    double *dP0 = (double *)bP.p, *dP1 = dP0 + kSpMaxGroups * 12;
    int *dF = (int *)bF.p;
    hipStream_t st = s->stream;
    const dim3 gvec((unsigned)((n_pad + kSpWG - 1) / kSpWG)), bwg(kSpWG);
    const int groups = (int)std::min<int64_t>(kSpMaxGroups, (n_pad + kSpWG - 1) / kSpWG);
    const dim3 ggrp((unsigned)groups);
    const Affine3 ident = {{0, 0, 0}, {1, 0, 0, 0, 1, 0, 0, 0, 1}, 1.0};
    double sums[12];
    auto fetch_sums = [&]() -> int {
        BB_HIP_CHECK(hipStreamSynchronize(st));
        BB_HIP_CHECK(hipMemcpy(sums, dS, sizeof(sums), hipMemcpyDeviceToHost));
        return BB_OK;
    };
    auto orthonormalise = [&]() -> int {
        BB_HIP_CHECK(bb::launch(sp_affine_stats_kernel<double>, ggrp, bwg, 0, st, (const double *)dZ, dV,
                                n, n_pad, (const double *)dP1, groups, (int)kSpChol, 1.0, dF, dP0));
        BB_HIP_CHECK(bb::launch(sp_affine_centre_kernel<T>, gvec, bwg, 0, st, (const double *)dV, dV,
                                s->d_mv_in.as<T>(), n, n_pad, (const double *)dP0, groups, dF));
        return BB_OK;
    };
    auto apply_B = [&]() -> int {
        BB_TRY(launch_grad(s, kOpMatvec2, s->d_mv_in.p));
        BB_TRY(exchange_sum(s));
        BB_HIP_CHECK(bb::launch(sp_stats_kernel<T>, ggrp, bwg, 0, st, (const T *)s->d_exch, n, n_pad, dP0));
        BB_HIP_CHECK(bb::launch(sp_affine_stats_kernel<T>, ggrp, bwg, 0, st, (const T *)s->d_exch, dZ, n,
                                n_pad, (const double *)dP0, groups, (int)kSpMean, -0.5, dF, dP1));
        return BB_OK;
    };
    BB_HIP_CHECK(hipMemsetAsync(dF, 0, sizeof(int), st));
    BB_HIP_CHECK(hipMemsetAsync(s->d_V, 0, (size_t)n3 * sizeof(T), st));
    BB_HIP_CHECK(upload_padded(s, dZ, v0, st));
    BB_HIP_CHECK(bb::launch(sp_stats_kernel<double>, ggrp, bwg, 0, st, (const double *)dZ, n, n_pad, dP1));
    BB_TRY(orthonormalise());
// ... 315 lines not shown
```

blueberry_amd/csrc/bb_solver_kernels.h:

```cpp
#pragma once

#include <hip/hip_runtime.h>
#include <stdint.h>

#include <type_traits>

#include "blueberry_hip.h"

namespace {


template <typename T>
struct Traits;
template <>
struct Traits<float> {
    using Vec = float4;
    static constexpr int VPL = 4;
    static __device__ __forceinline__ float eps2() { return 1e-30f; }
};
template <>
struct Traits<double> {
    using Vec = double2;
    static constexpr int VPL = 2;
    static __device__ __forceinline__ double eps2() { return 1e-300; }
// ... 296 lines not shown
        }
        acc = __builtin_amdgcn_mfma_f64_16x16x4f64(gx, sel[3 * r + 0], acc, 0, 0, 0);
        acc = __builtin_amdgcn_mfma_f64_16x16x4f64(gy, sel[3 * r + 1], acc, 0, 0, 0);
        acc = __builtin_amdgcn_mfma_f64_16x16x4f64(gz, sel[3 * r + 2], acc, 0, 0, 0);
    }
    double t = (acc.x + acc.y) + (acc.z + acc.w);
    t = swap_sum16(t);
    t = swap_sum32(t);
    *reinterpret_cast<double *>(row_lds + stage_idx) = t;
    const u32x2 bits = {(unsigned)__double2loint(t), (unsigned)__double2hiint(t)};
    __builtin_amdgcn_raw_buffer_store_b64(bits, row_rsrc, row_voff, 0, 0);
    stress += s;
}

typedef float f32x2 __attribute__((ext_vector_type(2)));

struct StripF32 {
    f32x2 x[2][2][3];
    f32x2 g[2][2][3];
};

__device__ __forceinline__ f32x2 weight01(f32x2 delta) {
    f32x2 w;
    const f32x2 big = {0x1p100f, 0x1p100f};
    asm("v_pk_mul_f32 %0, %1, %2 clamp" : "=v"(w) : "v"(delta), "v"(big));
    return w;
}

template <int K, int H, bool FIRST, int OP>
__device__ __forceinline__ void pair_step2(f32x2 delta, f32x2 xi, f32x2 yi, f32x2 zi, StripF32 &st,
                                           f32x2 &rx, f32x2 &ry, f32x2 &rz, f32x2 &s2) {
    if constexpr (OP == kOpMatvec2) {
        const f32x2 a = delta * delta;
        if constexpr (FIRST) {
            rx = a * st.x[K][H][0]; ry = a * st.x[K][H][1]; rz = a * st.x[K][H][2];
        } else {
            rx += a * st.x[K][H][0]; ry += a * st.x[K][H][1]; rz += a * st.x[K][H][2];
        }
        st.g[K][H][0] += a * xi;
        st.g[K][H][1] += a * yi;
        st.g[K][H][2] += a * zi;
        return;
    }
    const f32x2 eps2 = {1e-30f, 1e-30f};
    const f32x2 dx = xi - st.x[K][H][0], dy = yi - st.x[K][H][1], dz = zi - st.x[K][H][2];
    const f32x2 d2 = dx * dx + (dy * dy + (dz * dz + eps2));
    f32x2 rinv;
    rinv.x = __builtin_amdgcn_rsqf(d2.x);
    rinv.y = __builtin_amdgcn_rsqf(d2.y);
    if constexpr (is_weighted_op<OP>()) {
        const f32x2 res = (d2 * rinv - delta) * weight01(delta);
        f32x2 a = delta;
        if constexpr (OP == kOpStressW2) a = delta * delta;
        f32x2 w;
        w.x = __builtin_amdgcn_rcpf(__builtin_fmaxf(a.x, 0x1p-126f));
        w.y = __builtin_amdgcn_rcpf(__builtin_fmaxf(a.y, 0x1p-126f));
        const f32x2 t = res * w;
        s2 += res * t;
        const f32x2 coef = t * rinv;
        if constexpr (FIRST) {
            rx = coef * dx; ry = coef * dy; rz = coef * dz;
        } else {
            rx += coef * dx; ry += coef * dy; rz += coef * dz;
        }
        st.g[K][H][0] -= coef * dx;
        st.g[K][H][1] -= coef * dy;
        st.g[K][H][2] -= coef * dz;
        return;
    }
    f32x2 res = d2 * rinv - delta;
    res *= weight01(delta);
    s2 += res * res;
    const f32x2 coef = res * rinv;
    if constexpr (FIRST) {
        rx = coef * dx; ry = coef * dy; rz = coef * dz;
    } else {
        rx += coef * dx; ry += coef * dy; rz += coef * dz;
    }
    st.g[K][H][0] -= coef * dx;
    st.g[K][H][1] -= coef * dy;
    st.g[K][H][2] -= coef * dz;
}

template <bool NT, int OP, typename WIN>
__device__ __forceinline__ void process_unit_f32(float4 (&d)[8], const float (&xrow)[12],
                                                 const WIN &next, StripF32 &st,
                                                 double &stress, __amdgpu_buffer_rsrc_t row_rsrc,
                                                 unsigned row_voff, int stage_idx) {
    extern __shared__ __attribute__((aligned(16))) float row_lds[];
    f32x2 s2 = {0.f, 0.f};
    float g[12], h[6], m[3];
    auto row = [&](auto rc) __attribute__((always_inline)) {
        constexpr int r = decltype(rc)::value;
        const float xs = xrow[3 * r], ys = xrow[3 * r + 1], zs = xrow[3 * r + 2];
        const f32x2 xi = {xs, xs}, yi = {ys, ys}, zi = {zs, zs};
        f32x2 rx, ry, rz;
        pair_step2<0, 0, true, OP>(f32x2{d[2 * r].x, d[2 * r].y}, xi, yi, zi, st, rx, ry, rz, s2);
        pair_step2<0, 1, false, OP>(f32x2{d[2 * r].z, d[2 * r].w}, xi, yi, zi, st, rx, ry, rz, s2);
        d[2 * r] = next.template load<NT>(2 * r);
        pair_step2<1, 0, false, OP>(f32x2{d[2 * r + 1].x, d[2 * r + 1].y}, xi, yi, zi, st, rx, ry, rz, s2);
        pair_step2<1, 1, false, OP>(f32x2{d[2 * r + 1].z, d[2 * r + 1].w}, xi, yi, zi, st, rx, ry, rz, s2);
        d[2 * r + 1] = next.template load<NT>(2 * r + 1);
        g[3 * r] = rx.x + rx.y; g[3 * r + 1] = ry.x + ry.y; g[3 * r + 2] = rz.x + rz.y;
        row_sums_step<r>(g, h, m);
    };
    row(std::integral_constant<int, 0>{});
    row(std::integral_constant<int, 1>{});
    row(std::integral_constant<int, 2>{});
    row(std::integral_constant<int, 3>{});
    const float keep = row16_sum3(m[0], m[1], m[2]);
    row_lds[stage_idx] = keep;
    __builtin_amdgcn_raw_buffer_store_b32(__float_as_uint(keep), row_rsrc, row_voff, 0, 0);
    stress += (double)(s2.x + s2.y);
}

__device__ __forceinline__ void load_strip(StripF32 &st, const float *__restrict__ X, int j0,
                                           int lane) {
#pragma unroll
    for (int k = 0; k < 2; ++k) {
        const float4 *p = reinterpret_cast<const float4 *>(
            X + ((int64_t)j0 + k * 256 + (int64_t)lane * 4) * 3);
        const float4 a = p[0], b = p[1], c = p[2];
        st.x[k][0][0] = f32x2{a.x, a.w}; st.x[k][0][1] = f32x2{a.y, b.x};
        st.x[k][0][2] = f32x2{a.z, b.y};
        st.x[k][1][0] = f32x2{b.z, c.y}; st.x[k][1][1] = f32x2{b.w, c.z};
        st.x[k][1][2] = f32x2{c.x, c.w};
#pragma unroll
        for (int h = 0; h < 2; ++h)
#pragma unroll
            for (int c3 = 0; c3 < 3; ++c3) st.g[k][h][c3] = f32x2{0.f, 0.f};
    }
}

__device__ __forceinline__ void store_strip(const StripF32 &st, float *__restrict__ slot,
                                            int lane) {
#pragma unroll
    for (int k = 0; k < 2; ++k) {
        float4 *p = reinterpret_cast<float4 *>(slot + (k * 256 + (int64_t)lane * 4) * 3);
        const auto &g = st.g[k];
        p[0] = make_float4(g[0][0].x, g[0][1].x, g[0][2].x, g[0][0].y);
        p[1] = make_float4(g[0][1].y, g[0][2].y, g[1][0].x, g[1][1].x);
        p[2] = make_float4(g[1][2].x, g[1][0].y, g[1][1].y, g[1][2].y);
    }
}

template <typename T>
__device__ __forceinline__ const typename Traits<T>::Vec *unit_ptr(const T *__restrict__ units,
                                                                   int64_t ul, int lane) {
    using Vec = typename Traits<T>::Vec;
    return reinterpret_cast<const Vec *>(units) + ul * 512 + lane;
}

template <typename T, bool W>
__device__ __forceinline__ T load_xrow(const T *__restrict__ X, int i0, int lane) {
    return X[(int64_t)i0 * 3 + (lane < 3 * Lay<T, W>::RPU ? lane : 0)];
}

template <int LPR>
struct StripF64 {
    double xj[LPR][2][3], gc[LPR][2][3];
};
template <int LPR>
__device__ __forceinline__ void load_strip(StripF64<LPR> &st, const double *__restrict__ X, int j0,
                                           int lane) {
#pragma unroll
    for (int k = 0; k < LPR; ++k) {
        const double2 *p =
            reinterpret_cast<const double2 *>(X + ((int64_t)j0 + k * 128 + (int64_t)lane * 2) * 3);
        const double2 a = p[0], b = p[1], c = p[2];
        st.xj[k][0][0] = a.x; st.xj[k][0][1] = a.y; st.xj[k][0][2] = b.x;
        st.xj[k][1][0] = b.y; st.xj[k][1][1] = c.x; st.xj[k][1][2] = c.y;
    }
#pragma unroll
    for (int k = 0; k < LPR; ++k)
#pragma unroll
        for (int c = 0; c < 2; ++c) st.gc[k][c][0] = st.gc[k][c][1] = st.gc[k][c][2] = 0.0;
}
template <int LPR>
__device__ __forceinline__ void store_strip(const StripF64<LPR> &st, double *__restrict__ slot,
                                            int lane) {
#pragma unroll
    for (int k = 0; k < LPR; ++k) {
        double2 *p = reinterpret_cast<double2 *>(slot + ((int64_t)k * 128 + (int64_t)lane * 2) * 3);
        const auto &g = st.gc[k];
        p[0] = make_double2(g[0][0], g[0][1]);
        p[1] = make_double2(g[0][2], g[1][0]);
        p[2] = make_double2(g[1][1], g[1][2]);
    }
}
template <typename T, bool W, bool NT, int OP, int WPB>
__global__ __launch_bounds__(64 * WPB, (Lay<T, W>::MIN_WG)) void stress_grad_kernel(
    const T *__restrict__ units, const T *__restrict__ X, const int2 *__restrict__ udesc,
    int chunk_q, int chunk_r, const int2 *__restrict__ wave_slots, T *__restrict__ rowpart,
    T *__restrict__ colpart, double *__restrict__ stresspart, int cap_units, int lds_wave_floats,
    int dense_u0, double *__restrict__ stress_slot) {
    using Vec = typename Traits<T>::Vec;
    constexpr int VW = Lay<T, W>::VW;
    constexpr bool DEFER = sizeof(T) == 4 || W;
    const int lane = threadIdx.x & 63;
    const int wib = __builtin_amdgcn_readfirstlane(threadIdx.x >> 6);
    const int wg = (int)blockIdx.x;
    const int w = wg * WPB + wib;
    const int ua = w * chunk_q + (w < chunk_r ? w : chunk_r);
    const int ub = ua + chunk_q + (w < chunk_r ? 1 : 0);
    double stress = 0.0;
    int ws_shared[WPB];
#pragma unroll
    for (int k = 0; k < WPB; ++k) ws_shared[k] = wave_slots[(int64_t)wg * WPB + k].y;
    extern __shared__ __attribute__((aligned(16))) float row_lds[];
    const int stage0 = wib * lds_wave_floats;
    int *progress = reinterpret_cast<int *>(row_lds + WPB * lds_wave_floats);
    int partner_done = 0;
    const int park_from = (ub - ua) > cap_units ? (ub - ua) - cap_units : 0;
    double sel[6];
#pragma unroll
    for (int v = 0; v < 6; ++v) sel[v] = (lane & 15) == v ? 1.0 : 0.0;

    if (ua < ub) {
        int slot = wave_slots[w].x;
        Vec d[8];
        using Strip = typename std::conditional<sizeof(T) == 4, StripF32,
                                                StripF64<Lay<T, W>::LPR>>::type;
        Strip st;
        auto strip_load = [&](int j0) __attribute__((always_inline)) { load_strip(st, X, j0, lane); };
        auto strip_store = [&](int sl) __attribute__((always_inline)) {
            store_strip(st, colpart + (int64_t)sl * (3 * VW), lane);
        };

        int2 dc;
        if (dense_u0 >= 0) {
            constexpr int UPT = VW / Lay<T, W>::RPU;
            const unsigned g = (unsigned)dense_u0 + (unsigned)ua;
            const unsigned t = g / UPT, sub = g % UPT;
            unsigned J = (unsigned)((__builtin_sqrtf(8.0f * (float)t + 1.0f) - 1.0f) * 0.5f);
            while (J * (J + 1) / 2 > t) --J;
            while ((J + 1) * (J + 2) / 2 <= t) ++J;
            const unsigned I = t - J * (J + 1) / 2;
            dc = make_int2((int)(I * VW + sub * Lay<T, W>::RPU), (int)(J * VW));
        } else {
            dc = udesc[ua];
        }
        int2 dn = udesc[ua + 1 < ub ? ua + 1 : ua];
        struct XRowS {
            T v[3 * Lay<T, W>::RPU];
            __device__ __forceinline__ T get(int q) const { return v[q]; }
        };
        struct XRowV {
            T v;
            __device__ __forceinline__ T get(int q) const { return lane_value(v, q); }
        };
        using XRow = typename std::conditional<Lay<T, W>::SCALAR_XROW, XRowS, XRowV>::type;
        auto xrow_load = [&](int i0) __attribute__((always_inline)) {
            XRow x;
            if constexpr (std::is_same<XRow, XRowS>::value) {
                const T *px = X + (int64_t)i0 * 3;
#pragma unroll
                for (int q = 0; q < 3 * Lay<T, W>::RPU; ++q) x.v[q] = px[q];
            } else {
                x.v = load_xrow<T, W>(X, i0, lane);
            }
            return x;
        };
        XRow xr = xrow_load(dc.x);
        using Win = WinPtr<Vec>;
        auto window_of = [&](int u_next) __attribute__((always_inline)) {
            const bool real = u_next < ub;
            return Win{unit_ptr<T>(units, real ? u_next : ub - 1, real ? lane : 0)};
        };
        {
            const Win first = window_of(ua);
#pragma unroll
            for (int r = 0; r < 8; ++r) d[r] = first.template load<NT>(r);
        }
        constexpr unsigned kRowBytes = 3 * Lay<T, W>::RPU * sizeof(T);
        const __amdgpu_buffer_rsrc_t row_rsrc = __builtin_amdgcn_make_buffer_rsrc(
            rowpart + (int64_t)ua * (3 * Lay<T, W>::RPU), 0, (int)((unsigned)(ub - ua) * kRowBytes),
            0x00020000);

        const int f32_sl12 = swap_rowsum_slot(lane);
        const unsigned f32_voff_lane = swap_rowsum_stores(lane) ? (unsigned)f32_sl12 * 4u : 0x40000000u;
        const int f32_lds_lane = stage0 + f32_sl12;
        auto unit_step = [&](int u) __attribute__((always_inline)) {
            if constexpr (WPB == 8) {
                const int mine = u - ua;
                if (__builtin_amdgcn_readfirstlane(partner_done) > mine)
                    __builtin_amdgcn_s_setprio(1);
                else
                    __builtin_amdgcn_s_setprio(0);
                __hip_atomic_store(progress + wib, mine, __ATOMIC_RELAXED, __HIP_MEMORY_SCOPE_WORKGROUP);
                partner_done = __hip_atomic_load(progress + (wib ^ 4), __ATOMIC_RELAXED,
                                                 __HIP_MEMORY_SCOPE_WORKGROUP);
            }
            const int un = u + 1 < ub ? u + 1 : u;
            const XRow xrn = xrow_load(dn.x);
            const int2 dnn = udesc[un + 1 < ub ? un + 1 : un];
            const int k = u - ua;
            const bool parked = k >= park_from;
            if constexpr (sizeof(T) == 4) {
                const unsigned row_voff =
                    f32_voff_lane + (parked ? 0x40000000u : (unsigned)k * kRowBytes);
                const int stage_slot = f32_lds_lane + (parked ? k - park_from : 0) * 12;
                float xs12[12];
#pragma unroll
                for (int q = 0; q < 12; ++q) xs12[q] = xr.get(q);
                process_unit_f32<NT, OP>(d, xs12, window_of(u + 1), st, stress, row_rsrc, row_voff,
                                         stage_slot);
            } else if constexpr (W) {
                const bool mine = lane >= 48 && lane < 54;
                const unsigned row_voff =
                    (mine && !parked) ? (unsigned)k * kRowBytes + (unsigned)(lane - 48) * 8u
                                      : kDropOffset;
                const int stage_slot =
                    stage0 + ((mine && parked) ? (k - park_from) * 12 + (lane - 48) * 2
                                               : cap_units * 12 + 2 * (lane & 1));
                process_unit_f64w<NT, OP>(d, xr, window_of(u + 1), st.xj, st.gc, sel, stress,
                                          row_rsrc, row_voff, stage_slot);
            } else {
                const unsigned row_voff = lane == 63 ? (unsigned)k * kRowBytes : kDropOffset;
                process_unit_f64n<NT, OP>(d, xr, window_of(u + 1), st.xj, st.gc, stress,
                                          row_rsrc, row_voff);
            }
            xr = xrn;
            dc = dn;
            dn = dnn;
        };
        int u = ua;
        for (;;) {
            const int curj = dc.y;
            strip_load(curj);
            __builtin_amdgcn_s_waitcnt(0x0F70);
            do {
                unit_step(u);
                ++u;
            } while (u < ub && dc.y == curj);
            if (u >= ub) break;
            strip_store(slot);
            {
                const double sv = wave_sum_hi(stress);
                if (lane == 63) stress_slot[slot] = sv;
                stress = 0.0;
            }
            ++slot;
        }
        if constexpr (WPB == 8) {
            __hip_atomic_store(progress + wib, 0x7fffffff, __ATOMIC_RELAXED, __HIP_MEMORY_SCOPE_WORKGROUP);
            __builtin_amdgcn_s_setprio(0);
        }
        if constexpr (DEFER) {
            __builtin_amdgcn_fence(__ATOMIC_ACQ_REL, "wavefront");
            __builtin_amdgcn_wave_barrier();
            const int n4 = ((ub - ua) - park_from) * 3;
            float4 *dst = reinterpret_cast<float4 *>(rowpart + ((int64_t)ua + park_from) *
                                                                   (3 * Lay<T, W>::RPU));
            const int lane_q = (int)__builtin_amdgcn_mbcnt_hi(~0u, __builtin_amdgcn_mbcnt_lo(~0u, 0u));
            for (int q = lane_q; q < n4; q += 64) {
                const float *src = row_lds + stage0 + 4 * q;
                dst[q] = make_float4(src[0], src[1], src[2], src[3]);
            }
            __builtin_amdgcn_fence(__ATOMIC_ACQ_REL, "wavefront");
            __builtin_amdgcn_wave_barrier();
        }
        store_strip(st, reinterpret_cast<T *>(row_lds + stage0), lane);
    }
    __builtin_amdgcn_fence(__ATOMIC_RELEASE, "workgroup", "local");
    __builtin_amdgcn_s_barrier();
    __builtin_amdgcn_fence(__ATOMIC_ACQUIRE, "workgroup", "local");
    {
        constexpr int CH = 3 * VW, NTH = 64 * WPB;
        int k = 0;
        while (k < WPB) {
            const int sl = ws_shared[k];
            if (sl < 0) { ++k; continue; }
            int k2 = k + 1;
            while (k2 < WPB && ws_shared[k2] == sl) ++k2;
            T *dst = colpart + (int64_t)sl * CH;
#pragma unroll
            for (int j = 0; j < (CH + NTH - 1) / NTH; ++j) {
                const int e = (int)threadIdx.x + NTH * j;
                if (CH % NTH == 0 || e < CH) {
                    T acc = T(0);
                    for (int q = k; q < k2; ++q)
                        acc += reinterpret_cast<const T *>(row_lds + q * lds_wave_floats)[e];
                    dst[e] = acc;
                }
            }
            k = k2;
        }
    }

    stress = wave_sum_hi(stress);
    if (lane == 63) stresspart[w] = stress;
}

enum ReduceMode {
    kReduceApply = 0,
    kReduceExchange = 1,
    kReduceStressOnly = 2,
    kReducePeer = 4
};

constexpr int kMaxPeers = 16;
template <typename T>
struct PeerTable {
    T *dst[kMaxPeers];
    unsigned long long *flag[kMaxPeers];
};
struct PeerState {
    int status;
    int pad;
    unsigned long long verdict;
    unsigned long long decided;
};
constexpr unsigned long long kPeerPoison = ~0ull;

template <typename T>
struct ReduceParams {
    const T *__restrict__ part;
    const double *__restrict__ stresspart;
    T *__restrict__ X;
    T *__restrict__ V;
    T mu;
    T scale;
    T *__restrict__ exch;
    const PeerTable<T> *__restrict__ peer;
    unsigned *__restrict__ peer_counter;
    const PeerState *peer_state;
    unsigned long long seq;
    int n_peers;
    double *__restrict__ stress_out;
    int64_t n_pad;
    int n_waves;
    int mode;
    T lr;
    const double *__restrict__ stress_slot;
    int n_slots;
    const T *__restrict__ bin_scale;
    const unsigned *__restrict__ peer_mask;
    int rank;
    const int *__restrict__ map_ptr;
    const int *__restrict__ map_idx;
    int n_maps;
};

template <typename T>
__device__ __forceinline__ double stress_share(const ReduceParams<T> &p, int m, int tid, int stride) {
    double s = 0.0;
    if (p.n_maps <= 1) {
        for (int i = tid; i < p.n_waves; i += stride) s += p.stresspart[i];
        for (int i = tid; i < p.n_slots; i += stride) s += p.stress_slot[i];
    } else {
        for (int i = p.map_ptr[m] + tid; i < p.map_ptr[m + 1]; i += stride) {
            const int idx = p.map_idx[i];
            s += idx < p.n_waves ? p.stresspart[idx] : p.stress_slot[idx - p.n_waves];
        }
    }
    return s;
}

constexpr int kRedWG = 128;

template <typename T>
__device__ __forceinline__ T momentum_velocity(T mu, T vo, T lr, T g) { return mu * vo - lr * g; }
template <typename T>
__device__ __forceinline__ void momentum_step(T *__restrict__ X, T *__restrict__ V, int64_t o, T xo, T vo,
                                              T mu, T lr, T g) {
    const T v = momentum_velocity(mu, vo, lr, g);
    V[o] = v;
    X[o] = xo + v;
}
template <typename T>
__device__ __forceinline__ void momentum_step(T *__restrict__ X, T *__restrict__ V, int64_t o, T mu, T lr,
                                              T g) {
    const T vo = V[o];
    momentum_step(X, V, o, X[o], vo, mu, lr, g);
// ... 732 lines not shown
            }
            if (lane == 0 && row > 0) atomicAdd(deg + i, row);
        }
    }
    flush();
}

template <typename T, bool W, int Q>
__global__ __launch_bounds__(256) void unit_weight_sums_kernel(const T *__restrict__ units,
                                                               const int2 *__restrict__ udesc,
                                                               int64_t n_local, int64_t n_bins,
                                                               double *__restrict__ sums) {
    constexpr int VW = Lay<T, W>::VW, RPU = Lay<T, W>::RPU;
    const int lane = threadIdx.x & 63;
    const int64_t i = (int64_t)blockIdx.x * 4 + (threadIdx.x >> 6);
    if (i >= n_bins) return;
    auto weight = [](T v) -> double {
        const double d = (double)v;
        return d > 0.0 ? (Q == 1 ? 1.0 / d : 1.0 / (d * d)) : 0.0;
    };
    auto lower = [&](int j0, int i0) -> int64_t {
        int64_t lo = 0, hi = n_local;
        while (lo < hi) {
            const int64_t mid = (lo + hi) >> 1;
            const int2 d = udesc[mid];
            if (d.y < j0 || (d.y == j0 && d.x < i0)) lo = mid + 1;
            else hi = mid;
        }
        return lo;
    };
    const int b = (int)(i / VW);
    const int n_blocks = (int)((n_bins + VW - 1) / VW);
    const int i0 = (int)(i - i % RPU), r = (int)(i % RPU);
    double acc = 0.0;
    for (int J = b; J < n_blocks; ++J) {
        const int64_t ul = lower(J * VW, i0);
        if (ul >= n_local || udesc[ul].y != J * VW || udesc[ul].x != i0) continue;
        const T *row = units + ul * (RPU * VW) + (int64_t)r * VW;
        for (int c = lane; c < VW; c += 64) {
            const int64_t j = (int64_t)J * VW + c;
            if (j > i && j < n_bins) acc += weight(row[c]);
        }
    }
    const int c = (int)(i - (int64_t)b * VW);
    for (int64_t p = lane; p * RPU < i; p += 64) {
        const int64_t ul = lower(b * VW, (int)(p * RPU));
        if (ul >= n_local || udesc[ul].y != b * VW || udesc[ul].x != (int)(p * RPU)) continue;
        const T *col = units + ul * (RPU * VW) + c;
        for (int q = 0; q < RPU; ++q)
            if (p * RPU + q < i) acc += weight(col[q * VW]);
    }
    acc = wave_sum_hi(acc);
    if (lane == 63) sums[i] = acc;
}

template <bool NT>
__global__ __launch_bounds__(256, 4) void stream_read_kernel(const float4 *__restrict__ units,
                                                             int chunk_q, int chunk_r,
                                                             float *__restrict__ sink) {
    const int lane = threadIdx.x & 63;
    const int w = __builtin_amdgcn_readfirstlane(blockIdx.x * 4 + (threadIdx.x >> 6));
    const int ua = w * chunk_q + (w < chunk_r ? w : chunk_r);
    const int ub = ua + chunk_q + (w < chunk_r ? 1 : 0);
    float4 acc = make_float4(0.f, 0.f, 0.f, 0.f);
    if (ua < ub) {
        float4 d[8];
        const float4 *first = units + (int64_t)ua * 512 + lane;
#pragma unroll
        for (int r = 0; r < 8; ++r) d[r] = stream_load<NT>(first + r * 64);
        for (int u = ua; u < ub; ++u) {
            const int un = u + 1 < ub ? u + 1 : u;
            const float4 *next = units + (int64_t)un * 512 + lane;
#pragma unroll
            for (int r = 0; r < 8; ++r) {
                acc.x += d[r].x; acc.y += d[r].y; acc.z += d[r].z; acc.w += d[r].w;
                d[r] = stream_load<NT>(next + r * 64);
                __builtin_amdgcn_sched_barrier(0);
            }
        }
    }
    if (acc.x + acc.y + acc.z + acc.w == 12345.678f) sink[w] = acc.x;
}

template <typename TA, typename TB>
__global__ __launch_bounds__(1024) void gram3_kernel(const TA *__restrict__ A,
                                                     const TB *__restrict__ B, int64_t n,
                                                     double *__restrict__ out) {
    __shared__ double sh[12][16];
    double acc[12];
#pragma unroll
    for (int q = 0; q < 12; ++q) acc[q] = 0.0;
    for (int64_t i = threadIdx.x; i < n; i += 1024) {
        const double a0 = (double)A[3 * i], a1 = (double)A[3 * i + 1], a2 = (double)A[3 * i + 2];
        const double b0 = (double)B[3 * i], b1 = (double)B[3 * i + 1], b2 = (double)B[3 * i + 2];
        acc[0] = fma(a0, b0, acc[0]); acc[1] = fma(a0, b1, acc[1]); acc[2] = fma(a0, b2, acc[2]);
        acc[3] = fma(a1, b0, acc[3]); acc[4] = fma(a1, b1, acc[4]); acc[5] = fma(a1, b2, acc[5]);
        acc[6] = fma(a2, b0, acc[6]); acc[7] = fma(a2, b1, acc[7]); acc[8] = fma(a2, b2, acc[8]);
        acc[9] += a0; acc[10] += a1; acc[11] += a2;
    }
    const int lane = threadIdx.x & 63, wv = threadIdx.x >> 6;
#pragma unroll
    for (int q = 0; q < 12; ++q) {
        double v = acc[q];
#pragma unroll
        for (int off = 32; off > 0; off >>= 1) v += __shfl_down(v, off, 64);
        if (lane == 0) sh[q][wv] = v;
    }
    __syncthreads();
    if (threadIdx.x < 12) {
        double v = 0.0;
        for (int k = 0; k < 16; ++k) v += sh[threadIdx.x][k];
        out[threadIdx.x] = v;
    }
}

struct Affine3 {
    double mean[3], m[9], scale;
};
template <typename TI, typename TO>
__global__ __launch_bounds__(256) void affine3_kernel(const TI *__restrict__ in, TO *__restrict__ out,
                                                      int64_t n_bins, int64_t n_pad, Affine3 a) {
    const int64_t i = (int64_t)blockIdx.x * 256 + threadIdx.x;
    if (i >= n_pad) return;
    double o0 = 0.0, o1 = 0.0, o2 = 0.0;
    if (i < n_bins) {
        const double x0 = (double)in[3 * i] - a.mean[0], x1 = (double)in[3 * i + 1] - a.mean[1],
                     x2 = (double)in[3 * i + 2] - a.mean[2];
        o0 = a.scale * (x0 * a.m[0] + x1 * a.m[3] + x2 * a.m[6]);
        o1 = a.scale * (x0 * a.m[1] + x1 * a.m[4] + x2 * a.m[7]);
        o2 = a.scale * (x0 * a.m[2] + x1 * a.m[5] + x2 * a.m[8]);
    }
    out[3 * i] = (TO)o0; out[3 * i + 1] = (TO)o1; out[3 * i + 2] = (TO)o2;
}

constexpr int kSpWG = 256;
constexpr int kSpMaxGroups = 256;

__device__ __forceinline__ void sp_rows(int64_t n_pad, int64_t &r0, int64_t &r1) {
    const int64_t per = (n_pad + gridDim.x - 1) / gridDim.x;
    r0 = (int64_t)blockIdx.x * per;
    r1 = r0 + per < n_pad ? r0 + per : n_pad;
}
__device__ __forceinline__ void sp_store_partial(double (&acc)[12], double *__restrict__ partial) {
    __shared__ double sh[12][kSpWG / 64];
    const int lane = threadIdx.x & 63, wv = threadIdx.x >> 6;
#pragma unroll
    for (int q = 0; q < 12; ++q) {
        double v = acc[q];
#pragma unroll
        for (int off = 32; off > 0; off >>= 1) v += __shfl_down(v, off, 64);
        if (lane == 0) sh[q][wv] = v;
    }
    __syncthreads();
    if (threadIdx.x < 12) {
        double v = 0.0;
#pragma unroll
        for (int k = 0; k < kSpWG / 64; ++k) v += sh[threadIdx.x][k];
        partial[(int64_t)blockIdx.x * 12 + threadIdx.x] = v;
    }
}
__device__ __forceinline__ void sp_accumulate(double (&acc)[12], double a0, double a1, double a2) {
    acc[0] = fma(a0, a0, acc[0]); acc[1] = fma(a0, a1, acc[1]); acc[2] = fma(a0, a2, acc[2]);
    acc[3] = fma(a1, a0, acc[3]); acc[4] = fma(a1, a1, acc[4]); acc[5] = fma(a1, a2, acc[5]);
    acc[6] = fma(a2, a0, acc[6]); acc[7] = fma(a2, a1, acc[7]); acc[8] = fma(a2, a2, acc[8]);
    acc[9] += a0; acc[10] += a1; acc[11] += a2;
}
// ... 158 lines not shown
```

blueberry_amd/solver.py:

```python
import contextlib
import os
import sys

import numpy

from . import _lib

_DTYPES = {"float32": _lib.BB_F32, "float64": _lib.BB_F64}
_KINDS = {"wish": _lib.BB_KIND_WISH, "counts": _lib.BB_KIND_COUNTS}


class RankDeficient(RuntimeError):
    """The block power iteration of the device-resident spectral start lost rank: the map has
    fewer than three independent directions (an empty or unconstrained map, fewer than 4 bins).
    `fit()` then takes the host-driven start; every other library error propagates."""


class DeviceTriples(object):
    is_triples = True

    def __init__(self, triples, resolution, device):
        t = _check_triples(triples)
        self.resolution = int(resolution)
        if t.flags.c_contiguous:
# ... 389 lines not shown
        ok = all(h is not None for h in handles)
        if ok:
            ok = self._lib.bb_solver_peer_connect(self._h, b"".join(handles)) == _lib.BB_OK
        if not ok:
            self._peer_error = _lib.last_error()
        oks = [None] * self.world
        dist.all_gather_object(oks, bool(ok))
        self._peer = all(oks)
        return self._peer

    def iterate_peer(self, iters, lr):
        self._call("iterate_peer", int(iters), float(lr))

    def sync_timeout(self, milliseconds):
        self._call("sync_timeout", int(milliseconds))

    def comm_abort(self):
        self._call("comm_abort")

    def peer_form(self):
        return "one launch" if self._get(_lib.c_int, "peer_form") else "two launches"

    def peer_set_form(self, one_launch):
        self._call("peer_set_form", 1 if one_launch else 0)

    def peer_set_timeout(self, milliseconds):
        self._call("peer_set_timeout", int(milliseconds))

    def comm_world(self):
        n = _lib.c_int()
        if self._lib.bb_solver_comm_world(self._h, n) != _lib.BB_OK:
            return None
        return int(n.value)

    def peer_status(self):
        return int(self._get(_lib.c_int, "peer_status"))

    def exchange_tensor(self):
        if self._exch is None:
            import torch
            rts = _lib.hip_runtimes_loaded()
            if len(rts) > 1:
                raise RuntimeError(
                    "two HIP runtimes are loaded (%s): import torch BEFORE the first "
                    "blueberry_amd compute call in a distributed job, so that "
                    "libblueberry_hip.so binds to the runtime torch uses" % ", ".join(rts))
            tdt = torch.float32 if self.dtype == "float32" else torch.float64
            dev = torch.device("cuda", self.device)
            self._exch = torch.zeros(self.exchange_size(), dtype=tdt, device=dev)
            stream = torch.cuda.current_stream(dev)
            self._call("set_stream", _lib.c_void_p(stream.cuda_stream))
            self._call("set_exchange_buffer", _lib.c_void_p(self._exch.data_ptr()))
        return self._exch

    def set_timing(self, enabled):
        self._call("set_timing", int(enabled))

    def timing(self):
        g, r, n = _lib.c_dbl(), _lib.c_dbl(), _lib.c_i64()
        self._call("get_timing", g, r, n)
        return {"grad_ms": float(g.value), "reduce_ms": float(r.value), "launches": int(n.value),
                "step_ms": float(self._get(_lib.c_dbl, "get_step_timing"))}

    def score_timing(self):
        t = [_lib.c_dbl() for _ in range(3)]
        self._call("get_score_timing", *t)
        return tuple(float(v.value) for v in t)

    def event_gap_ms(self, pairs=16):
        return float(self._get(_lib.c_dbl, "measure_event_gap", int(pairs)))

    def stream_read_ms(self, launches=10):
        return float(self._get(_lib.c_dbl, "measure_stream_read", int(launches)))

    def iteration_path(self):
        ro, wpr = _lib.c_int(), _lib.c_int()
        self._call("iteration_path", ro, wpr)
        return ("row_owner", int(wpr.value)) if ro.value else ("units", 0)

    def traffic(self):
        b, p = _lib.c_i64(), _lib.c_i64()
        self._call("traffic", b, p)
        return {"unit_bytes": int(b.value), "pairs_dense": int(p.value)}


class GroupEngine(object):

    def __init__(self, n_bins, dtype, devices, tiles=None):
        self._lib = _lib.load()
        self.n_bins, self.dtype = int(n_bins), dtype
        self.devices = [int(d) for d in devices]
        self.device = self.devices[0]
        self.world = 1
        self._comm_state = "group"
        self._g = _lib.c_void_p()
        self.members = []
        try:
            R = len(self.devices)
            for r, d in enumerate(self.devices):
                self.members.append(HipEngine(n_bins, dtype, rank=r, world=R, device=d, tiles=tiles))
            handles = (_lib.c_void_p * R)(*[m._h.value for m in self.members])
            _lib.check(self._lib.bb_group_create(self._g, handles, R), "bb_group_create")
        except BaseException:
            self.close()
            raise

    def close(self):
        if self._g:
            self._lib.bb_group_destroy(self._g)
            self._g = _lib.c_void_p()
        for m in self.members:
            m.close()
        self.members = []

    def __del__(self):
        try:
            self.close()
        except Exception:
            pass

    def _each(self, name, *args):
        for e in self.members:
            getattr(e, name)(*args)

    def _summed(self, name, *args):
        out = getattr(self.members[0], name)(*args)
        for e in self.members[1:]:
            out = out + getattr(e, name)(*args)
        return out

    def layout(self):
        return self.members[0].layout()

    def set_wish_dense(self, matrix, kind, alpha):
        self._each("set_wish_dense", _check_square(matrix, self.n_bins), kind, alpha)

    def set_wish_sparse(self, rows, cols, vals, kind, alpha, KRnorm=None, KRexpected=None):
        self._each("set_wish_sparse", rows, cols, vals, kind, alpha, KRnorm, KRexpected)

    def set_wish_triples(self, dev_triples, kind, alpha, KRnorm=None, KRexpected=None):
        per_device = getattr(dev_triples, "per_device", {dev_triples.device: dev_triples})
        for e in self.members:
            e.set_wish_triples(per_device[e.device], kind, alpha, KRnorm, KRexpected)

    def set_wish_from_coords(self, xstar):
        self._each("set_wish_from_coords", _check_coords(xstar, self.n_bins))

    def set_wish_resident(self, cm, kind, alpha):
        dev = cm._resident()
        host = None
        for e in self.members:
            if e.device == dev.device:
                e.set_wish_resident(cm, kind, alpha)
                continue
            rc = self._lib.bb_solver_set_wish_from_cm(e._h, dev._h, _KINDS[kind], float(alpha))
            if rc == _lib.BB_OK:
                continue
            if not (rc == _lib.BB_ERR_INVALID and "without peer access" in _lib.last_error()):
                _lib.check(rc, "bb_solver_set_wish_from_cm")
            if host is None:
                host = cm.to_host()
            e.set_wish_dense(host, kind, alpha)

    def degrees(self):
        return self._summed("degrees")

# ... 986 lines not shown
```

include/blueberry_hip.h:

```cpp
#ifndef BLUEBERRY_HIP_H
#define BLUEBERRY_HIP_H

#include <stdint.h>

#ifdef __cplusplus
extern "C" {
#endif

#define BB_API __attribute__((visibility("default")))

#define BB_VERSION 100

enum {
    BB_OK = 0,
    BB_ERR_INVALID = 1,
    BB_ERR_HIP = 2,
    BB_ERR_STATE = 3,
    BB_ERR_NOMEM = 4
};

enum { BB_F32 = 0, BB_F64 = 1 };
enum { BB_KIND_WISH = 0, BB_KIND_COUNTS = 1 };

BB_API int bb_version(void);
// ... 46 lines not shown
BB_API int bb_solver_stress_maps(bb_solver *s, double *stress, int n_maps);
BB_API int bb_solver_degrees(bb_solver *s, int64_t *degree, int64_t n_bins);
BB_API int bb_solver_set_bin_steps(bb_solver *s, const double *scale, int64_t n_bins);
BB_API int bb_solver_set_block_steps(bb_solver *s, const double *scale, int64_t n_blocks);
BB_API int bb_solver_set_weight_power(bb_solver *s, int q);
BB_API int bb_solver_weight_sums(bb_solver *s, double *sums, int64_t n_bins);
BB_API int bb_solver_set_wish_sparse(bb_solver *s, const int64_t *rows, const int64_t *cols,
                                     const double *vals, int64_t nnz, int kind, double alpha,
                                     const double *KRnorm, const double *KRexpected);
typedef struct bb_triples bb_triples;
BB_API int bb_triples_create(bb_triples **out, const double *triples, int64_t n, int32_t resolution,
                             int32_t row_major, int device);
BB_API int bb_triples_destroy(bb_triples *t);
BB_API int bb_triples_tiles(const bb_triples *t, int64_t n_bins, int dtype, uint8_t *present,
                            int64_t n_blocks);
BB_API int bb_solver_set_wish_triples(bb_solver *s, const bb_triples *t, int kind, double alpha,
                                      const double *KRnorm, const double *KRexpected);
BB_API int bb_solver_set_wish_from_coords(bb_solver *s, const double *xstar);

BB_API int bb_solver_set_coords(bb_solver *s, const double *xyz);
BB_API int bb_solver_get_coords(bb_solver *s, double *xyz);

BB_API int bb_solver_set_momentum(bb_solver *s, double mu);

BB_API int bb_solver_iterate(bb_solver *s, int64_t iters, double lr);

BB_API int bb_solver_grad(bb_solver *s);
BB_API int bb_solver_apply(bb_solver *s, double lr);
BB_API int bb_solver_exchange_size(const bb_solver *s, int64_t *n_elems);
BB_API int bb_solver_get_exchange_buffer(bb_solver *s, void **dev_ptr);
BB_API int bb_solver_set_exchange_buffer(bb_solver *s, void *dev_ptr);
BB_API int bb_comm_unique_id(void *id_out_128_bytes);
BB_API int bb_solver_comm_init(bb_solver *s, const void *unique_id_128_bytes);
BB_API int bb_solver_allreduce(bb_solver *s);
BB_API int bb_solver_iterate_dist(bb_solver *s, int64_t iters, double lr);
BB_API int bb_solver_comm_world(const bb_solver *s, int *world);
BB_API int bb_solver_comm_abort(bb_solver *s);
BB_API int bb_comm_cached(int device, int rank, int world, int *available);
BB_API int bb_comm_cached_generation(int device, int rank, int world, int *available,
                                     uint64_t *generation);
BB_API int bb_solver_comm_attach(bb_solver *s);
BB_API int bb_solver_comm_detach(bb_solver *s);
BB_API int bb_comm_cache_clear(void);

#define BB_PEER_HANDLE_BYTES 128
BB_API int bb_solver_peer_export(bb_solver *s, void *handle_out);
BB_API int bb_solver_peer_connect(bb_solver *s, const void *handles_rank_order);
BB_API int bb_solver_iterate_peer(bb_solver *s, int64_t iters, double lr);
BB_API int bb_solver_peer_status(bb_solver *s, int *status);
BB_API int bb_solver_peer_set_timeout(bb_solver *s, int64_t milliseconds);
BB_API int bb_solver_peer_form(bb_solver *s, int *one_launch);
BB_API int bb_solver_peer_set_form(bb_solver *s, int one_launch);

typedef struct bb_group bb_group;
BB_API int bb_group_create(bb_group **out, bb_solver *const *members, int n);
BB_API int bb_group_iterate(bb_group *g, int64_t iters, double lr);
BB_API int bb_group_destroy(bb_group *g);

BB_API int bb_solver_read_exchange(bb_solver *s, double *host, int64_t n);
BB_API int bb_solver_write_exchange(bb_solver *s, const double *host, int64_t n);

BB_API int bb_solver_matvec_sq(bb_solver *s, const double *x, double *y);

BB_API int bb_solver_spectral_init(bb_solver *s, int n_iter, const double *v0);

BB_API int bb_solver_spectral_init_tol(bb_solver *s, int n_iter, double tol, const double *v0,
                                       int *iters_done, double *residual);

BB_API int bb_solver_stress(bb_solver *s, double *stress);
BB_API int bb_solver_score(bb_solver *s, const double *xyz, double *profile, double *bins);
BB_API int bb_solver_get_score_timing(bb_solver *s, double *profile_ms, double *fold_ms,
                                      double *bins_ms);
BB_API int bb_solver_get_stress_history(bb_solver *s, double *out, int64_t cap, int64_t *n);
BB_API int bb_solver_sync(bb_solver *s);
BB_API int bb_solver_sync_timeout(bb_solver *s, int64_t milliseconds);

BB_API int bb_solver_set_timing(bb_solver *s, int enabled);
BB_API int bb_solver_get_timing(bb_solver *s, double *grad_ms_avg, double *reduce_ms_avg,
                                int64_t *launches);
BB_API int bb_solver_get_step_timing(bb_solver *s, double *step_ms_avg);
BB_API int bb_solver_measure_event_gap(bb_solver *s, int pairs, double *ms_avg);
BB_API int bb_solver_measure_stream_read(bb_solver *s, int launches, double *ms_avg);
BB_API int bb_solver_iteration_path(const bb_solver *s, int *row_owner, int *waves_per_row);
BB_API int bb_solver_traffic(const bb_solver *s, int64_t *unit_bytes, int64_t *pairs_dense);


typedef struct bb_cm bb_cm;
BB_API int bb_cm_create(bb_cm **out, int64_t d, int device);
BB_API int bb_cm_destroy(bb_cm *cm);
BB_API int bb_cm_dim(const bb_cm *cm, int64_t *d);
BB_API int bb_cm_device_ptr(const bb_cm *cm, const double **dev_matrix, int64_t *d, int *device);
BB_API int bb_cm_upload(bb_cm *cm, const double *matrix, int64_t ld);
BB_API int bb_cm_download(bb_cm *cm, double *matrix, int64_t ld);
BB_API int bb_cm_scatter(bb_cm *cm, const double *triples, int64_t n, int32_t resolution);
BB_API int bb_cm_scatter_ex(bb_cm *cm, const double *triples, int64_t n, int32_t resolution,
                            int32_t row_major, uint8_t *present, int32_t *on_grid);
BB_API int bb_cm_normalize(bb_cm *cm, int64_t n_bins, const double *KRnorm,
                           const double *KRexpected);
BB_API int bb_cm_marginals(bb_cm *cm, double *sums);
BB_API int bb_cm_filter(bb_cm *cm, double threshold, int64_t *d_new, uint8_t *keep_out);
BB_API int bb_cm_symv(bb_cm *cm, const double *x, double *y);
BB_API int bb_cm_eigenvector(bb_cm *cm, double *vec, double *eigenvalue, double tol,
                             int64_t max_matvecs, int64_t *matvecs_used, double *residual);
BB_API int bb_cm_correlation(bb_cm *cm, double *tflops);
BB_API int bb_cm_release_scratch(int device);
BB_API int bb_cm_shortest_paths(const bb_cm *src, bb_cm *dst, int kind, double alpha,
                                int64_t *unreachable_pairs);
BB_API int bb_cm_balance(bb_cm *cm, int64_t n_bins, int64_t ignore_diags, int64_t min_nnz, double tol,
                         int64_t max_iter, double row_sum, double *bias, uint8_t *masked,
                         int64_t *iterations, double *variance);
BB_API int bb_cm_expected(bb_cm *cm, int64_t n_bins, const double *bias, double *sums,
                          int64_t *counts);
BB_API int bb_triples_balance(bb_triples *t, int64_t n_bins, int64_t ignore_diags, int64_t min_nnz,
                              double tol, int64_t max_iter, double row_sum, double *bias,
                              uint8_t *masked, int64_t *iterations, double *variance);
BB_API int bb_triples_expected(bb_triples *t, int64_t n_bins, const double *bias, double *sums,
                               int64_t *counts);
BB_API int bb_triples_pairs(bb_triples *t, int64_t n_bins, int64_t *n_pairs);
typedef struct bb_sig bb_sig;
BB_API int bb_binomial_sf(const int64_t *k, double n, const double *p, double *out, int64_t m,
                          int device);
BB_API int bb_cm_significance(bb_cm *cm, int64_t n_bins, int64_t k_lo, int64_t k_hi,
                              const double *bias, double bias_lo, double bias_hi,
                              const double *prior_by_distance, double n_total, bb_sig **out);
BB_API int bb_triples_significance(bb_triples *t, int64_t n_bins, int64_t k_lo, int64_t k_hi,
                                   const double *bias, double bias_lo, double bias_hi,
                                   const double *prior_by_distance, double n_total, bb_sig **out);
BB_API int bb_sig_size(const bb_sig *s, int64_t *n_listed, int64_t *terms);
BB_API int bb_sig_read(const bb_sig *s, int32_t *row, int32_t *col, double *count, double *p);
BB_API int bb_sig_timing(const bb_sig *s, double *list_ms, double *p_ms);
BB_API int bb_sig_destroy(bb_sig *s);
BB_API int bb_solver_set_wish_from_cm(bb_solver *s, const bb_cm *cm, int kind, double alpha);
BB_API int bb_solver_set_wish_from_cm_block(bb_solver *s, const bb_cm *cm, int64_t bin_offset,
                                            int kind, double alpha);


BB_API int bb_contactmap_scatter(const double *triples, int64_t n, int32_t resolution,
                                 double *matrix, int64_t d, int device);
BB_API int bb_contactmap_normalize(double *matrix, int64_t n_bins, const double *KRnorm,
                                   const double *KRexpected, int device);


BB_API int bb_benjamini_hochberg(const double *p_values, int64_t d, int64_t n, double *q_values,
                                 int device);
BB_API int bb_downsample(const float *yp1, int64_t n1, float *yp5i, int64_t n5, int device);

#ifdef __cplusplus
}
#endif
#endif
```

Measured before the change: 1623.

## Pack f32 wish units into 24-bit offset streams for stress sweeps

Adds a packed storage format for f32 wish-distance units. Each unit whose float bit patterns fit within a 24-bit range of a per-unit base is stored as 6 KiB instead of the raw unit size, and the kernel decodes it with integer add and byte permute instructions. A per-unit table carries the stream offset and base. The stress kernel switches between packed and raw bodies so it streams fewer bytes from memory. By default the packing is enabled only when the nontemporal (large working set) path is active and the saving is big enough. This adds a one-time host-side pass and extra per-unit decode work.

```diff
diff --git a/blueberry_amd/_lib.py b/blueberry_amd/_lib.py
--- a/blueberry_amd/_lib.py
+++ b/blueberry_amd/_lib.py
@@ -92,6 +92,7 @@
     "bb_solver_measure_stream_read": (c_int, [c_void_p, c_int, p_dbl]),
     "bb_solver_iteration_path": (c_int, [c_void_p, ctypes.POINTER(c_int), ctypes.POINTER(c_int)]),
     "bb_solver_traffic": (c_int, [c_void_p, p_i64, p_i64]),
+    "bb_solver_stream_info": (c_int, [c_void_p, p_i64, p_i64, p_i64, p_i64]),
     "bb_cm_create": (c_int, [ctypes.POINTER(c_void_p), c_i64, c_int]),
     "bb_cm_destroy": (c_int, [c_void_p]),
     "bb_cm_dim": (c_int, [c_void_p, p_i64]),
diff --git a/blueberry_amd/csrc/bb_solver.hip b/blueberry_amd/csrc/bb_solver.hip
--- a/blueberry_amd/csrc/bb_solver.hip
+++ b/blueberry_amd/csrc/bb_solver.hip
@@ -101,6 +101,12 @@
     int ro_blocks = 0, ro_wpr = 1;
     int64_t ro_launches = 0;
 
+    int pk_mode = -1;
+    int64_t pk_min_run = 64;
+    bool pk_stale = true, pk_valid = false;
+    bb::DevBuf pk_stream, pk_table;
+    int64_t pk_packed = 0, pk_bytes = 0, pk_switches = 0;
+
     bool timing = false;
     int timing_stride = 1;
     int64_t timing_iter = 0;
@@ -114,6 +120,7 @@
 void comm_release(bb_solver *s, bool destroy);
 
 constexpr int64_t kHistCap = 1 << 20;
+constexpr int64_t kPk24MinRun = 64;
 constexpr size_t kMaxTimedLaunches = 4096;
 
 int check_kind_alpha(const char *who, int kind, double alpha) {
@@ -197,6 +204,12 @@
     if (s->n_local >= ((int64_t)1 << 31))
         return bb::fail(BB_ERR_INVALID, "bb_solver_create: more than 2^31 units on one rank");
     s->nontemporal = s->n_local * bb::kUnitBytes > ((int64_t)240 << 20);
+    {
+        const char *e = getenv("BB_PACK24");
+        s->pk_mode = e ? (atoi(e) != 0 ? 1 : 0) : -1;
+        const char *r = getenv("BB_PACK24_MIN_RUN");
+        s->pk_min_run = r ? std::max<int64_t>(1, atoll(r)) : kPk24MinRun;
+    }
     s->chunk_q = (int)(s->n_local / nw);
     s->chunk_r = (int)(s->n_local % nw);
     std::vector<int2> wave_range(nw);
@@ -364,11 +377,87 @@
     else return v == V ? f(std::integral_constant<int, V>{}) : with_int<Rest...>(v, f);
 }
 
+constexpr int64_t kPk24MinSavingDiv = 8;
+constexpr int64_t kPk24PackedKiB = 6, kPk24RawKiB = bb::kUnitBytes / 1024;
+
+int ensure_pk24(bb_solver *s) {
+    if (!s->pk_stale) return BB_OK;
+    s->pk_stale = false, s->pk_valid = false;
+    s->pk_packed = s->pk_bytes = s->pk_switches = 0;
+    const int64_t n = s->n_local;
+    const bool want = s->dtype == BB_F32 && n > 0 && s->pk_mode != 0 && s->peer_ranks_on_gpu <= 1 &&
+                      (s->pk_mode == 1 || s->nontemporal);
+    if (!want) {
+        s->pk_stream.reset(), s->pk_table.reset();
+        return BB_OK;
+    }
+    bb::DevBuf d_minmax;
+    if (d_minmax.alloc((size_t)n * sizeof(uint2)) != hipSuccess) return BB_OK;
+    BB_HIP_CHECK(bb::launch(pk24_minmax_kernel, dim3((unsigned)n), dim3(256), 0, s->stream,
+                            (const uint4 *)s->d_units, d_minmax.as<uint2>()));
+    std::vector<uint2> mm((size_t)n);
+    BB_HIP_CHECK(hipMemcpyAsync(mm.data(), d_minmax.p, (size_t)n * sizeof(uint2), hipMemcpyDeviceToHost,
+                                s->stream));
+    BB_HIP_CHECK(hipStreamSynchronize(s->stream));
+    std::vector<int4> table((size_t)n);
+    int64_t kib = 0, packed = 0, switches = 0;
+    for (int64_t a = 0; a < n;) {
+        const bool pk = mm[(size_t)a].y - mm[(size_t)a].x < (1u << 24);
+        int64_t b = a + 1;
+        while (b < n && (mm[(size_t)b].y - mm[(size_t)b].x < (1u << 24)) == pk) ++b;
+        const bool store_packed = pk && b - a >= s->pk_min_run;
+        for (int64_t u = a; u < b; ++u) {
+            table[(size_t)u] = make_int4(s->udesc[(size_t)u].x, s->udesc[(size_t)u].y,
+                                         (int)((uint32_t)kib | (store_packed ? 0x80000000u : 0u)),
+                                         store_packed ? (int)mm[(size_t)u].x : 0);
+            kib += store_packed ? kPk24PackedKiB : kPk24RawKiB;
+        }
+        if (store_packed) packed += b - a;
+        a = b;
+    }
+    for (int64_t u = 1; u < n; ++u) switches += (table[(size_t)u].z < 0) != (table[(size_t)u - 1].z < 0);
+    const int64_t raw_kib = n * kPk24RawKiB;
+    const bool pays = s->pk_mode == 1 ? packed > 0 : kib * kPk24MinSavingDiv <= raw_kib * (kPk24MinSavingDiv - 1);
+    if (!pays || kib >= ((int64_t)1 << 31)) {
+        s->pk_stream.reset(), s->pk_table.reset();
+        return BB_OK;
+    }
+    if (s->pk_stream.reserve((size_t)(kib + kPk24RawKiB) * 1024) != hipSuccess ||
+        s->pk_table.reserve((size_t)n * sizeof(int4)) != hipSuccess) {
+        s->pk_stream.reset(), s->pk_table.reset();
+        return BB_OK;
+    }
+    BB_HIP_CHECK(hipMemcpyAsync(s->pk_table.p, table.data(), (size_t)n * sizeof(int4), hipMemcpyHostToDevice,
+                                s->stream));
+    BB_HIP_CHECK(hipMemsetAsync(s->pk_stream.as<char>() + kib * 1024, 0, (size_t)kPk24RawKiB * 1024, s->stream));
+    BB_HIP_CHECK(bb::launch(pk24_pack_kernel, dim3((unsigned)n), dim3(256), 0, s->stream,
+                            (const uint4 *)s->d_units, s->pk_table.as<const int4>(), s->pk_stream.as<uint4>()));
+    BB_HIP_CHECK(hipStreamSynchronize(s->stream));
+    s->pk_valid = true;
+    s->pk_packed = packed, s->pk_bytes = kib * 1024, s->pk_switches = switches;
+    return BB_OK;
+}
+
+template <bool NT, int OP, int WPB, bool PK, typename T, bool W>
+int launch_sweep_pk(LayoutTag<T, W>, bb_solver *s, const void *x_in);
+
 template <bool NT, int OP, int WPB, typename T, bool W>
-int launch_sweep(LayoutTag<T, W>, bb_solver *s, const void *x_in) {
-    const auto kern = stress_grad_kernel<T, W, NT, OP, WPB>;
+int launch_sweep(LayoutTag<T, W> lay, bb_solver *s, const void *x_in) {
+    if constexpr (sizeof(T) == 4 && OP == kOpStress) {
+        BB_TRY(ensure_pk24(s));
+        if (s->pk_valid) return launch_sweep_pk<NT, OP, WPB, true>(lay, s, x_in);
+    }
+    return launch_sweep_pk<NT, OP, WPB, false>(lay, s, x_in);
+}
+
+template <bool NT, int OP, int WPB, bool PK, typename T, bool W>
+int launch_sweep_pk(LayoutTag<T, W>, bb_solver *s, const void *x_in) {
+    const auto kern = [] {
+        if constexpr (PK) return stream24_grad_kernel<T, W, NT, OP, WPB>;
+        else return stress_grad_kernel<T, W, NT, OP, WPB>;
+    }();
     constexpr unsigned bit = 1u << ((WPB == 8 ? 4 : 0) + (NT ? 2 : 0) + (OP == kOpMatvec2 ? 1 : 0) +
-                                    (OP == kOpStressW1 ? 8 : 0) + (OP == kOpStressW2 ? 16 : 0));
+                                    (OP == kOpStressW1 ? 8 : 0) + (OP == kOpStressW2 ? 16 : 0) + (PK ? 24 : 0));
     if (s->defer_lds_bytes > 0 && !(s->defer_attr_done & bit)) {
         BB_HIP_CHECK(hipFuncSetAttribute((const void *)kern, hipFuncAttributeMaxDynamicSharedMemorySize,
                                          (int)s->defer_lds_bytes));
@@ -378,7 +467,8 @@
                  (s->u_begin - s->t_first * s->L.units_per_tile) * (3 * s->L.rows_per_unit);
     T *colpart = (T *)s->d_part + s->rowpart_elems;
     BB_HIP_CHECK(bb::launch(kern, dim3(s->n_waves / s->wpb), dim3(64 * s->wpb), (size_t)s->defer_lds_bytes,
-                            s->stream, (const T *)s->d_units, (const T *)x_in, s->d_udesc, s->chunk_q,
+                            s->stream, PK ? s->pk_stream.as<const T>() : (const T *)s->d_units,
+                            (const T *)x_in, PK ? s->pk_table.as<const int2>() : s->d_udesc, s->chunk_q,
                             s->chunk_r, s->d_wave_slots, rowpart, colpart, s->d_stresspart,
                             s->defer_cap_units, s->lds_wave_floats, s->dense_u0, s->d_stress_slot));
     return BB_OK;
@@ -640,12 +730,14 @@
 int inputs_done(bb_solver *s) {
     BB_HIP_CHECK(hipStreamSynchronize(s->stream));
     BB_TRY(refresh_full(s));
+    s->pk_stale = true;
     s->have_wish = true;
     return BB_OK;
 }
 
 int pack_from_cm(bb_solver *s, const double *m, int64_t d, int64_t off, int kind, double alpha) {
     BB_TRY(bb::enter_device(s->device));
+    s->pk_stale = true;
     if (s->n_local > 0)
         BB_TRY(by_layout(s, [&](auto lay) -> int {
             using T = typename decltype(lay)::T;
@@ -660,6 +752,7 @@
 int set_wish_dense(bb_solver *s, const double *host, int64_t ld, int kind, double alpha, int64_t off,
                    int64_t n_sub) {
     BB_TRY(bb::enter_device(s->device));
+    s->pk_stale = true;
     BB_TRY(by_layout(s, [&](auto lay) { return set_wish_dense_t(lay, s, host, ld, kind, alpha, off, n_sub); }));
     return inputs_done(s);
 }
@@ -683,6 +776,7 @@
         BB_TRY(hip(hipMemcpyAsync(bkr.p, KRnorm, (size_t)s->L.n_bins * 8, hipMemcpyHostToDevice, st)));
         BB_TRY(hip(hipMemcpyAsync(bke.p, KRexpected, (size_t)s->L.n_bins * 8, hipMemcpyHostToDevice, st)));
     }
+    s->pk_stale = true;
     BB_TRY(hip(hipMemsetAsync(bbad.p, 0, sizeof(int), st)));
     BB_TRY(hip(hipMemsetAsync(s->d_units, 0, (size_t)std::max<int64_t>(s->n_local, 1) * bb::kUnitBytes, st)));
     for (int64_t k0 = 0; k0 < n; k0 += chunk) {
@@ -931,6 +1025,7 @@
     BB_TRY(bb::alloc_status(s->d_map_scalar, (size_t)n_maps * sizeof(double)));
     BB_HIP_CHECK(hipMemcpy(s->d_map_ptr.p, ptr.data(), ptr.size() * sizeof(int), hipMemcpyHostToDevice));
     BB_HIP_CHECK(hipMemcpy(s->d_map_idx.p, idx.data(), idx.size() * sizeof(int), hipMemcpyHostToDevice));
+    s->pk_stale = true;
     BB_HIP_CHECK(hipMemsetAsync(s->d_units, 0, (size_t)std::max<int64_t>(s->n_local, 1) * bb::kUnitBytes,
                                 s->stream));
     BB_HIP_CHECK(hipStreamSynchronize(s->stream));
@@ -1231,6 +1326,7 @@
     BB_REQUIRE(s != nullptr && xstar != nullptr, "bb_solver_set_wish_from_coords: NULL argument");
     BB_TRY(bb::enter_device(s->device));
     BB_HIP_CHECK(upload_padded(s, s->d_f64_tmp, xstar, s->stream));
+    s->pk_stale = true;
     if (s->n_local > 0)
         BB_TRY(by_layout(s, [&](auto lay) -> int {
             using T = typename decltype(lay)::T;
@@ -1693,6 +1789,7 @@
         const char *env = getenv("BB_PEER_FUSED");
         s->peer_fused = env ? atoi(env) != 0 : most_on_one_gpu == 1;
         s->peer_ranks_on_gpu = most_on_one_gpu;
+        if (most_on_one_gpu > 1) s->pk_stale = true;
     }
     s->peer_connected = true;
     BB_HIP_CHECK(hipDeviceSynchronize());
@@ -2002,7 +2099,13 @@
     bb::Event e0, e1;
     BB_HIP_CHECK(e0.create());
     BB_HIP_CHECK(e1.create());
+    if (s->dtype == BB_F32) BB_TRY(ensure_pk24(s));
     auto launch = [&]() {
+        if (s->pk_valid)
+            return bb::launch(s->nontemporal ? stream_read_pk24_kernel<true> : stream_read_pk24_kernel<false>,
+                              dim3(s->n_waves / 4), dim3(256), 0, s->stream, s->pk_stream.as<const float4>(),
+                              s->pk_table.as<const int4>(), (int)s->n_local, (int)(s->pk_bytes / 1024),
+                              s->chunk_q, s->chunk_r, (float *)s->d_f64_tmp);
         return bb::launch(s->nontemporal ? stream_read_kernel<true> : stream_read_kernel<false>,
                           dim3(s->n_waves / 4), dim3(256), 0, s->stream,
                           (const float4 *)s->d_units, s->chunk_q, s->chunk_r,
@@ -2019,6 +2122,20 @@
     return BB_OK;
 }
 
+int bb_solver_stream_info(bb_solver *s, int64_t *packed_units, int64_t *raw_units, int64_t *stream_bytes,
+                          int64_t *format_switches) {
+    BB_REQUIRE(s != nullptr, "bb_solver_stream_info: solver is NULL");
+    if (!s->have_wish)
+        return bb::fail(BB_ERR_STATE, "bb_solver_stream_info: no wish distances set");
+    BB_TRY(bb::enter_device(s->device));
+    BB_TRY(ensure_pk24(s));
+    if (packed_units) *packed_units = s->pk_valid ? s->pk_packed : 0;
+    if (raw_units) *raw_units = s->pk_valid ? s->n_local - s->pk_packed : s->n_local;
+    if (stream_bytes) *stream_bytes = s->pk_valid ? s->pk_bytes : 0;
+    if (format_switches) *format_switches = s->pk_valid ? s->pk_switches : 0;
+    return BB_OK;
+}
+
 int bb_solver_iteration_path(const bb_solver *s, int *row_owner, int *waves_per_row) {
     BB_REQUIRE(s != nullptr, "bb_solver_iteration_path: solver is NULL");
     if (row_owner) *row_owner = s->row_owner ? 1 : 0;
@@ -2026,9 +2143,13 @@
     return BB_OK;
 }
 
-int bb_solver_traffic(const bb_solver *s, int64_t *unit_bytes, int64_t *pairs_dense) {
+int bb_solver_traffic(bb_solver *s, int64_t *unit_bytes, int64_t *pairs_dense) {
     BB_REQUIRE(s != nullptr, "bb_solver_traffic: solver is NULL");
-    if (unit_bytes) *unit_bytes = s->n_local * bb::kUnitBytes;
+    if (s->have_wish && s->dtype == BB_F32) {
+        BB_TRY(bb::enter_device(s->device));
+        BB_TRY(ensure_pk24(s));
+    }
+    if (unit_bytes) *unit_bytes = s->pk_valid && !s->pk_stale ? s->pk_bytes : s->n_local * bb::kUnitBytes;
     if (pairs_dense) *pairs_dense = s->L.n_bins * (s->L.n_bins - 1) / 2;
     return BB_OK;
 }
diff --git a/blueberry_amd/csrc/bb_solver_kernels.h b/blueberry_amd/csrc/bb_solver_kernels.h
--- a/blueberry_amd/csrc/bb_solver_kernels.h
+++ b/blueberry_amd/csrc/bb_solver_kernels.h
@@ -402,11 +402,37 @@
     st.g[K][H][2] -= coef * dz;
 }
 
-template <bool NT, int OP, typename WIN>
+template <bool ROW3>
+__device__ __forceinline__ void pk24_decode(float &word, unsigned base) {
+    if constexpr (ROW3) {
+        asm volatile("v_add_u32 %0, %0, %1" : "+v"(word) : "s"(base));
+    } else {
+        asm volatile("v_mad_u32_u24 %0, %0, 1, %1" : "+v"(word) : "s"(base));
+    }
+}
+template <bool ROW3>
+__device__ __forceinline__ void pk24_decode(float4 &w, unsigned base) {
+    pk24_decode<ROW3>(w.x, base); pk24_decode<ROW3>(w.y, base);
+    pk24_decode<ROW3>(w.z, base); pk24_decode<ROW3>(w.w, base);
+}
+constexpr unsigned kPk24SelPair = 0x0c0c0703u;
+constexpr unsigned kPk24SelThird = 0x0c070100u;
+__device__ __forceinline__ float pk24_tops(float hi, float lo, unsigned sel) {
+    float v;
+    asm volatile("v_perm_b32 %0, %1, %2, %3" : "=v"(v) : "v"(hi), "v"(lo), "s"(sel));
+    return v;
+}
+__device__ __forceinline__ float4 pk24_tops(float4 hi, float4 lo, unsigned sel) {
+    return make_float4(pk24_tops(hi.x, lo.x, sel), pk24_tops(hi.y, lo.y, sel),
+                       pk24_tops(hi.z, lo.z, sel), pk24_tops(hi.w, lo.w, sel));
+}
+
+template <bool NT, int OP, bool PK = false, typename WIN>
 __device__ __forceinline__ void process_unit_f32(float4 (&d)[8], const float (&xrow)[12],
                                                  const WIN &next, StripF32 &st,
                                                  double &stress, __amdgpu_buffer_rsrc_t row_rsrc,
-                                                 unsigned row_voff, int stage_idx) {
+                                                 unsigned row_voff, int stage_idx,
+                                                 unsigned base = 0u) {
     extern __shared__ __attribute__((aligned(16))) float row_lds[];
     f32x2 s2 = {0.f, 0.f};
     float g[12], h[6], m[3];
@@ -415,6 +441,30 @@
         const float xs = xrow[3 * r], ys = xrow[3 * r + 1], zs = xrow[3 * r + 2];
         const f32x2 xi = {xs, xs}, yi = {ys, ys}, zi = {zs, zs};
         f32x2 rx, ry, rz;
+        if constexpr (PK) {
+            constexpr int A = r < 3 ? 2 * r : 6, B = r == 0 ? 1 : (r == 1 ? 2 : (r == 2 ? 5 : 7));
+            if constexpr (r == 0) d[6] = pk24_tops(d[1], d[0], kPk24SelPair);
+            if constexpr (r == 1) d[6] = pk24_tops(d[2], d[6], kPk24SelThird);
+            if constexpr (r == 2) {
+                d[7] = pk24_tops(d[3], pk24_tops(d[5], d[4], kPk24SelPair), kPk24SelThird);
+                d[3] = next.template load<NT>(3);
+            }
+            pk24_decode<r == 3>(d[A], base);
+            pair_step2<0, 0, true, OP>(f32x2{d[A].x, d[A].y}, xi, yi, zi, st, rx, ry, rz, s2);
+            pair_step2<0, 1, false, OP>(f32x2{d[A].z, d[A].w}, xi, yi, zi, st, rx, ry, rz, s2);
+            if constexpr (r == 0) d[0] = next.template load<NT>(0);
+            if constexpr (r == 2) d[4] = next.template load<NT>(4);
+            if constexpr (r == 1) d[2] = d[3];
+            pk24_decode<r == 3>(d[B], base);
+            pair_step2<1, 0, false, OP>(f32x2{d[B].x, d[B].y}, xi, yi, zi, st, rx, ry, rz, s2);
+            pair_step2<1, 1, false, OP>(f32x2{d[B].z, d[B].w}, xi, yi, zi, st, rx, ry, rz, s2);
+            if constexpr (r == 0) d[1] = next.template load<NT>(1);
+            if constexpr (r == 1) d[2] = next.template load<NT>(2);
+            if constexpr (r == 2) d[5] = next.template load<NT>(5);
+            g[3 * r] = rx.x + rx.y; g[3 * r + 1] = ry.x + ry.y; g[3 * r + 2] = rz.x + rz.y;
+            row_sums_step<r>(g, h, m);
+            return;
+        }
         pair_step2<0, 0, true, OP>(f32x2{d[2 * r].x, d[2 * r].y}, xi, yi, zi, st, rx, ry, rz, s2);
         pair_step2<0, 1, false, OP>(f32x2{d[2 * r].z, d[2 * r].w}, xi, yi, zi, st, rx, ry, rz, s2);
         d[2 * r] = next.template load<NT>(2 * r);
@@ -508,208 +558,32 @@
         p[2] = make_double2(g[1][1], g[1][2]);
     }
 }
+__device__ __forceinline__ int64_t pk24_word_offset(const int4 &e) { return (int64_t)(e.z & 0x7fffffff) * 64; }
+__device__ __forceinline__ int64_t pk24_word_offset(const int2 &) { return 0; }
+__device__ __forceinline__ bool pk24_packed(const int4 &e) { return e.z < 0; }
+__device__ __forceinline__ bool pk24_packed(const int2 &) { return false; }
+__device__ __forceinline__ unsigned pk24_base(const int4 &e) { return (unsigned)e.w; }
+__device__ __forceinline__ unsigned pk24_base(const int2 &) { return 0u; }
+
 template <typename T, bool W, bool NT, int OP, int WPB>
 __global__ __launch_bounds__(64 * WPB, (Lay<T, W>::MIN_WG)) void stress_grad_kernel(
     const T *__restrict__ units, const T *__restrict__ X, const int2 *__restrict__ udesc,
     int chunk_q, int chunk_r, const int2 *__restrict__ wave_slots, T *__restrict__ rowpart,
     T *__restrict__ colpart, double *__restrict__ stresspart, int cap_units, int lds_wave_floats,
     int dense_u0, double *__restrict__ stress_slot) {
-    using Vec = typename Traits<T>::Vec;
-    constexpr int VW = Lay<T, W>::VW;
-    constexpr bool DEFER = sizeof(T) == 4 || W;
-    const int lane = threadIdx.x & 63;
-    const int wib = __builtin_amdgcn_readfirstlane(threadIdx.x >> 6);
-    const int wg = (int)blockIdx.x;
-    const int w = wg * WPB + wib;
-    const int ua = w * chunk_q + (w < chunk_r ? w : chunk_r);
-    const int ub = ua + chunk_q + (w < chunk_r ? 1 : 0);
-    double stress = 0.0;
-    int ws_shared[WPB];
-#pragma unroll
-    for (int k = 0; k < WPB; ++k) ws_shared[k] = wave_slots[(int64_t)wg * WPB + k].y;
-    extern __shared__ __attribute__((aligned(16))) float row_lds[];
-    const int stage0 = wib * lds_wave_floats;
-    int *progress = reinterpret_cast<int *>(row_lds + WPB * lds_wave_floats);
-    int partner_done = 0;
-    const int park_from = (ub - ua) > cap_units ? (ub - ua) - cap_units : 0;
-    double sel[6];
-#pragma unroll
-    for (int v = 0; v < 6; ++v) sel[v] = (lane & 15) == v ? 1.0 : 0.0;
-
-    if (ua < ub) {
-        int slot = wave_slots[w].x;
-        Vec d[8];
-        using Strip = typename std::conditional<sizeof(T) == 4, StripF32,
-                                                StripF64<Lay<T, W>::LPR>>::type;
-        Strip st;
-        auto strip_load = [&](int j0) __attribute__((always_inline)) { load_strip(st, X, j0, lane); };
-        auto strip_store = [&](int sl) __attribute__((always_inline)) {
-            store_strip(st, colpart + (int64_t)sl * (3 * VW), lane);
-        };
-
-        int2 dc;
-        if (dense_u0 >= 0) {
-            constexpr int UPT = VW / Lay<T, W>::RPU;
-            const unsigned g = (unsigned)dense_u0 + (unsigned)ua;
-            const unsigned t = g / UPT, sub = g % UPT;
-            unsigned J = (unsigned)((__builtin_sqrtf(8.0f * (float)t + 1.0f) - 1.0f) * 0.5f);
-            while (J * (J + 1) / 2 > t) --J;
-            while ((J + 1) * (J + 2) / 2 <= t) ++J;
-            const unsigned I = t - J * (J + 1) / 2;
-            dc = make_int2((int)(I * VW + sub * Lay<T, W>::RPU), (int)(J * VW));
-        } else {
-            dc = udesc[ua];
-        }
-        int2 dn = udesc[ua + 1 < ub ? ua + 1 : ua];
-        struct XRowS {
-            T v[3 * Lay<T, W>::RPU];
-            __device__ __forceinline__ T get(int q) const { return v[q]; }
-        };
-        struct XRowV {
-            T v;
-            __device__ __forceinline__ T get(int q) const { return lane_value(v, q); }
-        };
-        using XRow = typename std::conditional<Lay<T, W>::SCALAR_XROW, XRowS, XRowV>::type;
-        auto xrow_load = [&](int i0) __attribute__((always_inline)) {
-            XRow x;
-            if constexpr (std::is_same<XRow, XRowS>::value) {
-                const T *px = X + (int64_t)i0 * 3;
-#pragma unroll
-                for (int q = 0; q < 3 * Lay<T, W>::RPU; ++q) x.v[q] = px[q];
-            } else {
-                x.v = load_xrow<T, W>(X, i0, lane);
-            }
-            return x;
-        };
-        XRow xr = xrow_load(dc.x);
-        using Win = WinPtr<Vec>;
-        auto window_of = [&](int u_next) __attribute__((always_inline)) {
-            const bool real = u_next < ub;
-            return Win{unit_ptr<T>(units, real ? u_next : ub - 1, real ? lane : 0)};
-        };
-        {
-            const Win first = window_of(ua);
-#pragma unroll
-            for (int r = 0; r < 8; ++r) d[r] = first.template load<NT>(r);
-        }
-        constexpr unsigned kRowBytes = 3 * Lay<T, W>::RPU * sizeof(T);
-        const __amdgpu_buffer_rsrc_t row_rsrc = __builtin_amdgcn_make_buffer_rsrc(
-            rowpart + (int64_t)ua * (3 * Lay<T, W>::RPU), 0, (int)((unsigned)(ub - ua) * kRowBytes),
-            0x00020000);
-
-        const int f32_sl12 = swap_rowsum_slot(lane);
-        const unsigned f32_voff_lane = swap_rowsum_stores(lane) ? (unsigned)f32_sl12 * 4u : 0x40000000u;
-        const int f32_lds_lane = stage0 + f32_sl12;
-        auto unit_step = [&](int u) __attribute__((always_inline)) {
-            if constexpr (WPB == 8) {
-                const int mine = u - ua;
-                if (__builtin_amdgcn_readfirstlane(partner_done) > mine)
-                    __builtin_amdgcn_s_setprio(1);
-                else
-                    __builtin_amdgcn_s_setprio(0);
-                __hip_atomic_store(progress + wib, mine, __ATOMIC_RELAXED, __HIP_MEMORY_SCOPE_WORKGROUP);
-                partner_done = __hip_atomic_load(progress + (wib ^ 4), __ATOMIC_RELAXED,
-                                                 __HIP_MEMORY_SCOPE_WORKGROUP);
-            }
-            const int un = u + 1 < ub ? u + 1 : u;
-            const XRow xrn = xrow_load(dn.x);
-            const int2 dnn = udesc[un + 1 < ub ? un + 1 : un];
-            const int k = u - ua;
-            const bool parked = k >= park_from;
-            if constexpr (sizeof(T) == 4) {
-                const unsigned row_voff =
-                    f32_voff_lane + (parked ? 0x40000000u : (unsigned)k * kRowBytes);
-                const int stage_slot = f32_lds_lane + (parked ? k - park_from : 0) * 12;
-                float xs12[12];
-#pragma unroll
-                for (int q = 0; q < 12; ++q) xs12[q] = xr.get(q);
-                process_unit_f32<NT, OP>(d, xs12, window_of(u + 1), st, stress, row_rsrc, row_voff,
-                                         stage_slot);
-            } else if constexpr (W) {
-                const bool mine = lane >= 48 && lane < 54;
-                const unsigned row_voff =
-                    (mine && !parked) ? (unsigned)k * kRowBytes + (unsigned)(lane - 48) * 8u
-                                      : kDropOffset;
-                const int stage_slot =
-                    stage0 + ((mine && parked) ? (k - park_from) * 12 + (lane - 48) * 2
-                                               : cap_units * 12 + 2 * (lane & 1));
-                process_unit_f64w<NT, OP>(d, xr, window_of(u + 1), st.xj, st.gc, sel, stress,
-                                          row_rsrc, row_voff, stage_slot);
-            } else {
-                const unsigned row_voff = lane == 63 ? (unsigned)k * kRowBytes : kDropOffset;
-                process_unit_f64n<NT, OP>(d, xr, window_of(u + 1), st.xj, st.gc, stress,
-                                          row_rsrc, row_voff);
-            }
-            xr = xrn;
-            dc = dn;
-            dn = dnn;
-        };
-        int u = ua;
-        for (;;) {
-            const int curj = dc.y;
-            strip_load(curj);
-            __builtin_amdgcn_s_waitcnt(0x0F70);
-            do {
-                unit_step(u);
-                ++u;
-            } while (u < ub && dc.y == curj);
-            if (u >= ub) break;
-            strip_store(slot);
-            {
-                const double sv = wave_sum_hi(stress);
-                if (lane == 63) stress_slot[slot] = sv;
-                stress = 0.0;
-            }
-            ++slot;
-        }
-        if constexpr (WPB == 8) {
-            __hip_atomic_store(progress + wib, 0x7fffffff, __ATOMIC_RELAXED, __HIP_MEMORY_SCOPE_WORKGROUP);
-            __builtin_amdgcn_s_setprio(0);
-        }
-        if constexpr (DEFER) {
-            __builtin_amdgcn_fence(__ATOMIC_ACQ_REL, "wavefront");
-            __builtin_amdgcn_wave_barrier();
-            const int n4 = ((ub - ua) - park_from) * 3;
-            float4 *dst = reinterpret_cast<float4 *>(rowpart + ((int64_t)ua + park_from) *
-                                                                   (3 * Lay<T, W>::RPU));
-            const int lane_q = (int)__builtin_amdgcn_mbcnt_hi(~0u, __builtin_amdgcn_mbcnt_lo(~0u, 0u));
-            for (int q = lane_q; q < n4; q += 64) {
-                const float *src = row_lds + stage0 + 4 * q;
-                dst[q] = make_float4(src[0], src[1], src[2], src[3]);
-            }
-            __builtin_amdgcn_fence(__ATOMIC_ACQ_REL, "wavefront");
-            __builtin_amdgcn_wave_barrier();
-        }
-        store_strip(st, reinterpret_cast<T *>(row_lds + stage0), lane);
-    }
-    __builtin_amdgcn_fence(__ATOMIC_RELEASE, "workgroup", "local");
-    __builtin_amdgcn_s_barrier();
-    __builtin_amdgcn_fence(__ATOMIC_ACQUIRE, "workgroup", "local");
-    {
-        constexpr int CH = 3 * VW, NTH = 64 * WPB;
-        int k = 0;
-        while (k < WPB) {
-            const int sl = ws_shared[k];
-            if (sl < 0) { ++k; continue; }
-            int k2 = k + 1;
-            while (k2 < WPB && ws_shared[k2] == sl) ++k2;
-            T *dst = colpart + (int64_t)sl * CH;
-#pragma unroll
-            for (int j = 0; j < (CH + NTH - 1) / NTH; ++j) {
-                const int e = (int)threadIdx.x + NTH * j;
-                if (CH % NTH == 0 || e < CH) {
-                    T acc = T(0);
-                    for (int q = k; q < k2; ++q)
-                        acc += reinterpret_cast<const T *>(row_lds + q * lds_wave_floats)[e];
-                    dst[e] = acc;
-                }
-            }
-            k = k2;
-        }
-    }
-
-    stress = wave_sum_hi(stress);
-    if (lane == 63) stresspart[w] = stress;
+    constexpr bool PK = sizeof(T) == 0;
+#include "bb_sweep_body.inc"
+}
+
+template <typename T, bool W, bool NT, int OP, int WPB>
+__global__ __launch_bounds__(64 * WPB, (WPB == 8 ? 2 : 1)) void stream24_grad_kernel(
+    const T *__restrict__ units, const T *__restrict__ X, const int2 *__restrict__ udesc,
+    int chunk_q, int chunk_r, const int2 *__restrict__ wave_slots, T *__restrict__ rowpart,
+    T *__restrict__ colpart, double *__restrict__ stresspart, int cap_units, int lds_wave_floats,
+    int dense_u0, double *__restrict__ stress_slot) {
+    static_assert(sizeof(T) == 4 && W, "the 24-bit stream is fp32 only");
+    constexpr bool PK = sizeof(T) == 4;
+#include "bb_sweep_body.inc"
 }
 
 enum ReduceMode {
@@ -1608,6 +1482,79 @@
     if (acc.x + acc.y + acc.z + acc.w == 12345.678f) sink[w] = acc.x;
 }
 
+__global__ __launch_bounds__(256) void pk24_minmax_kernel(const uint4 *__restrict__ units,
+                                                          uint2 *__restrict__ minmax) {
+    __shared__ unsigned lo_s[4], hi_s[4];
+    const uint4 *p = units + (int64_t)blockIdx.x * 512 + threadIdx.x;
+    const uint4 a = p[0], b = p[256];
+    unsigned lo = min(min(min(a.x, a.y), min(a.z, a.w)), min(min(b.x, b.y), min(b.z, b.w)));
+    unsigned hi = max(max(max(a.x, a.y), max(a.z, a.w)), max(max(b.x, b.y), max(b.z, b.w)));
+    for (int o = 32; o > 0; o >>= 1) {
+        lo = min(lo, (unsigned)__shfl_xor((int)lo, o));
+        hi = max(hi, (unsigned)__shfl_xor((int)hi, o));
+    }
+    if ((threadIdx.x & 63) == 0) lo_s[threadIdx.x >> 6] = lo, hi_s[threadIdx.x >> 6] = hi;
+    __syncthreads();
+    if (threadIdx.x == 0)
+        minmax[blockIdx.x] = make_uint2(min(min(lo_s[0], lo_s[1]), min(lo_s[2], lo_s[3])),
+                                        max(max(hi_s[0], hi_s[1]), max(hi_s[2], hi_s[3])));
+}
+
+__global__ __launch_bounds__(256) void pk24_pack_kernel(const uint4 *__restrict__ units,
+                                                        const int4 *__restrict__ table,
+                                                        uint4 *__restrict__ stream) {
+    const int4 e = table[blockIdx.x];
+    const uint4 *src = units + (int64_t)blockIdx.x * 512;
+    uint4 *dst = stream + (int64_t)(e.z & 0x7fffffff) * 64;
+    const int t = threadIdx.x;
+    if (e.z >= 0) {
+        dst[t] = src[t];
+        dst[t + 256] = src[t + 256];
+        return;
+    }
+    const unsigned base = (unsigned)e.w;
+    for (int L = t >> 6; L < 6; L += 4) {
+        const int l = t & 63;
+        const int k3 = L < 3 ? 0 : 1;
+        const int sh = 8 * (L < 3 ? L : (L == 3 ? 2 : L - 4));
+        const uint4 w = src[L * 64 + l], r3 = src[(6 + k3) * 64 + l];
+        dst[L * 64 + l] = make_uint4((w.x - base) | ((((r3.x - base) >> sh) & 0xffu) << 24),
+                                     (w.y - base) | ((((r3.y - base) >> sh) & 0xffu) << 24),
+                                     (w.z - base) | ((((r3.z - base) >> sh) & 0xffu) << 24),
+                                     (w.w - base) | ((((r3.w - base) >> sh) & 0xffu) << 24));
+    }
+}
+
+template <bool NT>
+__global__ __launch_bounds__(256, 4) void stream_read_pk24_kernel(const float4 *__restrict__ stream,
+                                                                  const int4 *__restrict__ table,
+                                                                  int n_units, int end_kib,
+                                                                  int chunk_q, int chunk_r,
+                                                                  float *__restrict__ sink) {
+    const int lane = threadIdx.x & 63;
+    const int w = __builtin_amdgcn_readfirstlane(blockIdx.x * 4 + (threadIdx.x >> 6));
+    const int ua = w * chunk_q + (w < chunk_r ? w : chunk_r);
+    const int ub = ua + chunk_q + (w < chunk_r ? 1 : 0);
+    float4 acc = make_float4(0.f, 0.f, 0.f, 0.f);
+    if (ua < ub) {
+        const int ka = table[ua].z & 0x7fffffff;
+        const int kb = ub < n_units ? table[ub].z & 0x7fffffff : end_kib;
+        float4 d[8];
+        const float4 *base = stream + lane;
+#pragma unroll
+        for (int r = 0; r < 8; ++r) d[r] = stream_load<NT>(base + (int64_t)min(ka + r, kb - 1) * 64);
+        for (int k = ka; k < kb; k += 8) {
+#pragma unroll
+            for (int r = 0; r < 8; ++r) {
+                acc.x += d[r].x; acc.y += d[r].y; acc.z += d[r].z; acc.w += d[r].w;
+                d[r] = stream_load<NT>(base + (int64_t)min(k + 8 + r, kb - 1) * 64);
+                __builtin_amdgcn_sched_barrier(0);
+            }
+        }
+    }
+    if (acc.x + acc.y + acc.z + acc.w == 12345.678f) sink[w] = acc.x;
+}
+
 template <typename TA, typename TB>
 __global__ __launch_bounds__(1024) void gram3_kernel(const TA *__restrict__ A,
                                                      const TB *__restrict__ B, int64_t n,
diff --git a/blueberry_amd/csrc/bb_sweep_body.inc b/blueberry_amd/csrc/bb_sweep_body.inc
--- /dev/null
+++ b/blueberry_amd/csrc/bb_sweep_body.inc
@@ -0,0 +1,252 @@
+    using Vec = typename Traits<T>::Vec;
+    constexpr int VW = Lay<T, W>::VW;
+    constexpr bool DEFER = sizeof(T) == 4 || W;
+    const int lane = threadIdx.x & 63;
+    const int wib = __builtin_amdgcn_readfirstlane(threadIdx.x >> 6);
+    const int wg = (int)blockIdx.x;
+    const int w = wg * WPB + wib;
+    const int ua = w * chunk_q + (w < chunk_r ? w : chunk_r);
+    const int ub = ua + chunk_q + (w < chunk_r ? 1 : 0);
+    double stress = 0.0;
+    int ws_shared[WPB];
+#pragma unroll
+    for (int k = 0; k < WPB; ++k) ws_shared[k] = wave_slots[(int64_t)wg * WPB + k].y;
+    extern __shared__ __attribute__((aligned(16))) float row_lds[];
+    const int stage0 = wib * lds_wave_floats;
+    int *progress = reinterpret_cast<int *>(row_lds + WPB * lds_wave_floats);
+    int partner_done = 0;
+    const int park_from = (ub - ua) > cap_units ? (ub - ua) - cap_units : 0;
+    double sel[6];
+#pragma unroll
+    for (int v = 0; v < 6; ++v) sel[v] = (lane & 15) == v ? 1.0 : 0.0;
+
+    if (ua < ub) {
+        int slot = wave_slots[w].x;
+        Vec d[8];
+        using Strip = typename std::conditional<sizeof(T) == 4, StripF32,
+                                                StripF64<Lay<T, W>::LPR>>::type;
+        Strip st;
+        auto strip_load = [&](int j0) __attribute__((always_inline)) { load_strip(st, X, j0, lane); };
+        auto strip_store = [&](int sl) __attribute__((always_inline)) {
+            store_strip(st, colpart + (int64_t)sl * (3 * VW), lane);
+        };
+
+        using Desc = typename std::conditional<PK, int4, int2>::type;
+        const Desc *__restrict__ const table = reinterpret_cast<const Desc *>(udesc);
+        Desc dc;
+        if (dense_u0 >= 0) {
+            constexpr int UPT = VW / Lay<T, W>::RPU;
+            const unsigned g = (unsigned)dense_u0 + (unsigned)ua;
+            const unsigned t = g / UPT, sub = g % UPT;
+            unsigned J = (unsigned)((__builtin_sqrtf(8.0f * (float)t + 1.0f) - 1.0f) * 0.5f);
+            while (J * (J + 1) / 2 > t) --J;
+            while ((J + 1) * (J + 2) / 2 <= t) ++J;
+            const unsigned I = t - J * (J + 1) / 2;
+            if constexpr (PK) {
+                dc = table[ua];
+                dc.x = (int)(I * VW + sub * Lay<T, W>::RPU), dc.y = (int)(J * VW);
+            } else {
+                dc = make_int2((int)(I * VW + sub * Lay<T, W>::RPU), (int)(J * VW));
+            }
+        } else {
+            dc = table[ua];
+        }
+        Desc dn = table[ua + 1 < ub ? ua + 1 : ua];
+        struct XRowS {
+            T v[3 * Lay<T, W>::RPU];
+            __device__ __forceinline__ T get(int q) const { return v[q]; }
+        };
+        struct XRowV {
+            T v;
+            __device__ __forceinline__ T get(int q) const { return lane_value(v, q); }
+        };
+        using XRow = typename std::conditional<Lay<T, W>::SCALAR_XROW, XRowS, XRowV>::type;
+        auto xrow_load = [&](int i0) __attribute__((always_inline)) {
+            XRow x;
+            if constexpr (std::is_same<XRow, XRowS>::value) {
+                const T *px = X + (int64_t)i0 * 3;
+#pragma unroll
+                for (int q = 0; q < 3 * Lay<T, W>::RPU; ++q) x.v[q] = px[q];
+            } else {
+                x.v = load_xrow<T, W>(X, i0, lane);
+            }
+            return x;
+        };
+        XRow xr = xrow_load(dc.x);
+        using Win = WinPtr<Vec>;
+        auto window_of = [&](int u_next) __attribute__((always_inline)) {
+            const bool real = u_next < ub;
+            if constexpr (PK) {
+                return Win{reinterpret_cast<const Vec *>(units) + pk24_word_offset(dn) +
+                           (real ? lane : 0)};
+            } else {
+                return Win{unit_ptr<T>(units, real ? u_next : ub - 1, real ? lane : 0)};
+            }
+        };
+        auto window_here = [&]() __attribute__((always_inline)) {
+            return Win{reinterpret_cast<const Vec *>(units) + pk24_word_offset(dc) + lane};
+        };
+        if constexpr (PK) {
+            const Win first = window_here();
+#pragma unroll
+            for (int r = 0; r < 6; ++r) d[r] = first.template load<NT>(r);
+        } else {
+            const Win first = window_of(ua);
+#pragma unroll
+            for (int r = 0; r < 8; ++r) d[r] = first.template load<NT>(r);
+        }
+        constexpr unsigned kRowBytes = 3 * Lay<T, W>::RPU * sizeof(T);
+        const __amdgpu_buffer_rsrc_t row_rsrc = __builtin_amdgcn_make_buffer_rsrc(
+            rowpart + (int64_t)ua * (3 * Lay<T, W>::RPU), 0, (int)((unsigned)(ub - ua) * kRowBytes),
+            0x00020000);
+
+        const int f32_sl12 = swap_rowsum_slot(lane);
+        const unsigned f32_voff_lane = swap_rowsum_stores(lane) ? (unsigned)f32_sl12 * 4u : 0x40000000u;
+        const int f32_lds_lane = stage0 + f32_sl12;
+        auto unit_step = [&](int u, auto packed_body) __attribute__((always_inline)) {
+            if constexpr (WPB == 8) {
+                const int mine = u - ua;
+                if (__builtin_amdgcn_readfirstlane(partner_done) > mine)
+                    __builtin_amdgcn_s_setprio(1);
+                else
+                    __builtin_amdgcn_s_setprio(0);
+                __hip_atomic_store(progress + wib, mine, __ATOMIC_RELAXED, __HIP_MEMORY_SCOPE_WORKGROUP);
+                partner_done = __hip_atomic_load(progress + (wib ^ 4), __ATOMIC_RELAXED,
+                                                 __HIP_MEMORY_SCOPE_WORKGROUP);
+            }
+            const int un = u + 1 < ub ? u + 1 : u;
+            const XRow xrn = xrow_load(dn.x);
+            const Desc dnn = table[un + 1 < ub ? un + 1 : un];
+            const int k = u - ua;
+            const bool parked = k >= park_from;
+            if constexpr (sizeof(T) == 4) {
+                const unsigned row_voff =
+                    f32_voff_lane + (parked ? 0x40000000u : (unsigned)k * kRowBytes);
+                const int stage_slot = f32_lds_lane + (parked ? k - park_from : 0) * 12;
+                float xs12[12];
+#pragma unroll
+                for (int q = 0; q < 12; ++q) xs12[q] = xr.get(q);
+                if constexpr (decltype(packed_body)::value) {
+                    process_unit_f32<NT, OP, true>(d, xs12, window_of(u + 1), st, stress, row_rsrc,
+                                                   row_voff, stage_slot, pk24_base(dc));
+                } else {
+                    process_unit_f32<NT, OP>(d, xs12, window_of(u + 1), st, stress, row_rsrc, row_voff,
+                                             stage_slot);
+                }
+            } else if constexpr (W) {
+                const bool mine = lane >= 48 && lane < 54;
+                const unsigned row_voff =
+                    (mine && !parked) ? (unsigned)k * kRowBytes + (unsigned)(lane - 48) * 8u
+                                      : kDropOffset;
+                const int stage_slot =
+                    stage0 + ((mine && parked) ? (k - park_from) * 12 + (lane - 48) * 2
+                                               : cap_units * 12 + 2 * (lane & 1));
+                process_unit_f64w<NT, OP>(d, xr, window_of(u + 1), st.xj, st.gc, sel, stress,
+                                          row_rsrc, row_voff, stage_slot);
+            } else {
+                const unsigned row_voff = lane == 63 ? (unsigned)k * kRowBytes : kDropOffset;
+                process_unit_f64n<NT, OP>(d, xr, window_of(u + 1), st.xj, st.gc, stress,
+                                          row_rsrc, row_voff);
+            }
+            xr = xrn;
+            dc = dn;
+            dn = dnn;
+        };
+        int u = ua;
+        if constexpr (PK) {
+            for (;;) {
+                const int curj = dc.y;
+                strip_load(curj);
+                for (;;) {
+                    if (pk24_packed(dc)) {
+                        __builtin_amdgcn_s_waitcnt(0x0F70);
+                        do {
+                            unit_step(u, std::true_type{});
+                            ++u;
+                        } while (u < ub && dc.y == curj && pk24_packed(dc));
+                    } else {
+                        const Win here = window_here();
+                        d[6] = here.template load<NT>(6);
+                        d[7] = here.template load<NT>(7);
+                        __builtin_amdgcn_s_waitcnt(0x0F70);
+                        do {
+                            unit_step(u, std::false_type{});
+                            ++u;
+                        } while (u < ub && dc.y == curj && !pk24_packed(dc));
+                    }
+                    if (u >= ub || dc.y != curj) break;
+                }
+                if (u >= ub) break;
+                strip_store(slot);
+                const double sv = wave_sum_hi(stress);
+                if (lane == 63) stress_slot[slot] = sv;
+                stress = 0.0;
+                ++slot;
+            }
+        } else {
+            for (;;) {
+                const int curj = dc.y;
+                strip_load(curj);
+                __builtin_amdgcn_s_waitcnt(0x0F70);
+                do {
+                    unit_step(u, std::false_type{});
+                    ++u;
+                } while (u < ub && dc.y == curj);
+                if (u >= ub) break;
+                strip_store(slot);
+                {
+                    const double sv = wave_sum_hi(stress);
+                    if (lane == 63) stress_slot[slot] = sv;
+                    stress = 0.0;
+                }
+                ++slot;
+            }
+        }
+        if constexpr (WPB == 8) {
+            __hip_atomic_store(progress + wib, 0x7fffffff, __ATOMIC_RELAXED, __HIP_MEMORY_SCOPE_WORKGROUP);
+            __builtin_amdgcn_s_setprio(0);
+        }
+        if constexpr (DEFER) {
+            __builtin_amdgcn_fence(__ATOMIC_ACQ_REL, "wavefront");
+            __builtin_amdgcn_wave_barrier();
+            const int n4 = ((ub - ua) - park_from) * 3;
+            float4 *dst = reinterpret_cast<float4 *>(rowpart + ((int64_t)ua + park_from) *
+                                                                   (3 * Lay<T, W>::RPU));
+            const int lane_q = (int)__builtin_amdgcn_mbcnt_hi(~0u, __builtin_amdgcn_mbcnt_lo(~0u, 0u));
+            for (int q = lane_q; q < n4; q += 64) {
+                const float *src = row_lds + stage0 + 4 * q;
+                dst[q] = make_float4(src[0], src[1], src[2], src[3]);
+            }
+            __builtin_amdgcn_fence(__ATOMIC_ACQ_REL, "wavefront");
+            __builtin_amdgcn_wave_barrier();
+        }
+        store_strip(st, reinterpret_cast<T *>(row_lds + stage0), lane);
+    }
+    __builtin_amdgcn_fence(__ATOMIC_RELEASE, "workgroup", "local");
+    __builtin_amdgcn_s_barrier();
+    __builtin_amdgcn_fence(__ATOMIC_ACQUIRE, "workgroup", "local");
+    {
+        constexpr int CH = 3 * VW, NTH = 64 * WPB;
+        int k = 0;
+        while (k < WPB) {
+            const int sl = ws_shared[k];
+            if (sl < 0) { ++k; continue; }
+            int k2 = k + 1;
+            while (k2 < WPB && ws_shared[k2] == sl) ++k2;
+            T *dst = colpart + (int64_t)sl * CH;
+#pragma unroll
+            for (int j = 0; j < (CH + NTH - 1) / NTH; ++j) {
+                const int e = (int)threadIdx.x + NTH * j;
+                if (CH % NTH == 0 || e < CH) {
+                    T acc = T(0);
+                    for (int q = k; q < k2; ++q)
+                        acc += reinterpret_cast<const T *>(row_lds + q * lds_wave_floats)[e];
+                    dst[e] = acc;
+                }
+            }
+            k = k2;
+        }
+    }
+
+    stress = wave_sum_hi(stress);
+    if (lane == 63) stresspart[w] = stress;
diff --git a/blueberry_amd/solver.py b/blueberry_amd/solver.py
--- a/blueberry_amd/solver.py
+++ b/blueberry_amd/solver.py
@@ -495,6 +495,12 @@
         b, p = _lib.c_i64(), _lib.c_i64()
         self._call("traffic", b, p)
         return {"unit_bytes": int(b.value), "pairs_dense": int(p.value)}
+
+    def stream_info(self):
+        v = [_lib.c_i64() for _ in range(4)]
+        self._call("stream_info", *v)
+        return dict(zip(("packed_units", "raw_units", "stream_bytes", "format_switches"),
+                        (int(x.value) for x in v)))
 
 
 class GroupEngine(object):
diff --git a/include/blueberry_hip.h b/include/blueberry_hip.h
--- a/include/blueberry_hip.h
+++ b/include/blueberry_hip.h
@@ -152,7 +152,9 @@
 BB_API int bb_solver_measure_event_gap(bb_solver *s, int pairs, double *ms_avg);
 BB_API int bb_solver_measure_stream_read(bb_solver *s, int launches, double *ms_avg);
 BB_API int bb_solver_iteration_path(const bb_solver *s, int *row_owner, int *waves_per_row);
-BB_API int bb_solver_traffic(const bb_solver *s, int64_t *unit_bytes, int64_t *pairs_dense);
+BB_API int bb_solver_traffic(bb_solver *s, int64_t *unit_bytes, int64_t *pairs_dense);
+BB_API int bb_solver_stream_info(bb_solver *s, int64_t *packed_units, int64_t *raw_units,
+                                 int64_t *stream_bytes, int64_t *format_switches);
 
 
 typedef struct bb_cm bb_cm;
```

Measured after the change: 1731, median of 6. 1.07x the previous value.
